# SumitTarafder/Figbird

Hardware: AMD Instinct MI355X
Metric: gaps/sec (+ filled-bases/sec), synthetic 1e5-gap set recipe, jump-library fill pass (higher is better)
Workload: dtype f64

## Files before the change

figbird_amd/csrc/fig_abi.hip:

```cpp
#include <hip/hip_runtime.h>

#include <algorithm>
#include <cstdio>
#include <cstdlib>
#include <cstring>
#include <new>
#include <vector>
#include <chrono>
#include <thread>
#include <mutex>

#include "../../include/figbird_hip.h"
#include "fig_engine.h"
#include "fig_pack.h"
#include "fig_abi_host.h"
#include "fig_quality.h"
#include "fig_quality_host.h"

#ifdef FIG_PROF
#define FIG_PROF_BEGIN() const unsigned long long _k0 = __builtin_readcyclecounter()
#define FIG_PROF_FLUSH() do { if (E.lane == 0) { atomicAdd(&B.counters[FIG_CNT_WAIT], E.wait_cycles); atomicAdd(&B.counters[FIG_CNT_WAVE], (unsigned long long)__builtin_readcyclecounter() - _k0); \
    for (int i = 0; i < FIG_PROF_SLOTS; i++) if (E.prof[i]) atomicAdd(&B.counters[i < FIG_PROF_SPLIT ? FIG_CNT_PROF_LO + i : FIG_CNT_PROF_HI + (i - FIG_PROF_SPLIT)], E.prof[i]); } } while (0)
#else
#define FIG_PROF_BEGIN() ((void)0)
#define FIG_PROF_FLUSH() ((void)0)
#endif

FIG_D void fig_eng_init(FigEng &E, const FigDevModel &M, const FigDevBatch &B, const FigKernArgs &A, bool lds_tab, FigScr &work) {
    fig_eng_ident(E, threadIdx.x, blockDim.x, 64);
    E.M = &M; E.B = &B;
    E.flops = 0; E.mle_alg = 0; E.mle_exec = 0; E.wait_cycles = 0;
    for (int i = 0; i < FIG_PROF_SLOTS; i++) E.prof[i] = 0;
    unsigned char *slab = B.scratch + (long long)blockIdx.x * B.scratch_stride;
    fig_scratch_layout(slab, B.capG, B.capR, B.capP, B.capC, B.capW, B.capE, &work);
    E.scr = work;
    fig_eng_carve(E, M, A, lds_tab);
}

FIG_D void fig_kernel_begin(FigEng &E, const FigDevModel &M, const FigDevBatch &B, const FigKernArgs &A, bool lds_tab, FigScr &work) {
    fig_eng_init(E, M, B, A, lds_tab, work);
    if (blockIdx.x == 0 && threadIdx.x == 0) B.queue_head[A.qsel ^ 1] = 0;
}

FIG_D int fig_queue_pop(FigEng &E, const FigDevBatch &B, const FigKernArgs &A) {
    if (E.tid == 0) E.S->bc_i = atomicAdd(B.queue_head + A.qsel, 1);
    __syncthreads();
    const int qi = E.S->bc_i;
    __syncthreads();
    return qi;
}

template <typename T> struct FigItemSrc { const T *v; int first, end; };
FIG_D FigItemSrc<int32_t> fig_src_order(const FigDevBatch &B, const FigKernArgs &A) { return {B.order, A.q_begin, A.q_end}; }

template <typename Src, typename Body>
FIG_D void fig_pop_loop(FigEng &E, const FigDevBatch &B, const FigKernArgs &A, Src src, Body body) {
    while (true) {
        const int qi = fig_queue_pop(E, B, A);
        const auto s = src();
        if (s.first + qi >= s.end) break;
        body(s.v[s.first + qi]);
    }
}

FIG_D void fig_kernel_flush(const FigEng &E, const FigDevBatch &B) {
    if (E.flops) atomicAdd(&B.counters[FIG_CNT_FLOPS], E.flops);
    if (E.mle_alg) atomicAdd(&B.counters[FIG_CNT_MLE_ALG], E.mle_alg);
    if (E.lane == 0 && E.mle_exec) atomicAdd(&B.counters[FIG_CNT_MLE_EXEC], E.mle_exec);
}

template <bool LDS_TAB, int NT>
__global__ void __launch_bounds__(NT, (NT <= 256 ? 2 : 1)) fig_fill_kernel(FigDevModel M, FigDevBatch B, FigKernArgs A) {
    FigEng E; FigScr work;
    fig_kernel_begin(E, M, B, A, LDS_TAB, work);
    FIG_PROF_BEGIN();
    fig_pop_loop(E, B, A, [&] { return fig_src_order(B, A); }, [&](int gi) { fig_item_fill<LDS_TAB>(E, work, gi); });
    FIG_PROF_FLUSH();
    fig_kernel_flush(E, B);
}

template <bool LDS_TAB, int NT>
__global__ void __launch_bounds__(NT, (NT <= 256 ? 2 : 1)) fig_begin_kernel(FigDevModel M, FigDevBatch B, FigKernArgs A) {
    FigEng E; FigScr work;
    fig_kernel_begin(E, M, B, A, LDS_TAB, work);
    fig_pop_loop(E, B, A, [&] { return fig_src_order(B, A); }, [&](int gi) { fig_item_begin<LDS_TAB>(E, work, gi); });
    fig_kernel_flush(E, B);
}

template <bool LDS_TAB, int NT>
__global__ void __launch_bounds__(NT, (NT <= 256 ? 2 : 1)) fig_probe_kernel(FigDevModel M, FigDevBatch B, FigKernArgs A) {
    FigEng E; FigScr work;
    fig_kernel_begin(E, M, B, A, LDS_TAB, work);
    fig_pop_loop(E, B, A, [&] { return fig_src_order(B, A); }, [&](int gi) { fig_item_probe<LDS_TAB>(E, work, gi); });
}

static_assert(sizeof(FigItem) == sizeof(int4) && sizeof(FigEntry) == sizeof(int4), "item records travel as int4");
template <bool LDS_TAB, int NT>
__global__ void __launch_bounds__(NT, (NT <= 256 ? 2 : 1)) fig_eval_kernel(FigDevModel M, FigDevBatch B, FigKernArgs A, const int4 *items, int n_items) {
    FigEng E; FigScr work;
    fig_kernel_begin(E, M, B, A, LDS_TAB, work);
    FIG_PROF_BEGIN();
    fig_pop_loop(E, B, A, [&] { return FigItemSrc<FigItem>{(const FigItem *)items, 0, n_items}; }, [&](FigItem it) { fig_item_eval<LDS_TAB>(E, work, it); });
    FIG_PROF_FLUSH();
    fig_kernel_flush(E, B);
}

__global__ void __launch_bounds__(64) fig_replay_kernel(FigDevModel M, FigDevBatch B, const int4 *entries, int n) {
    if ((int)blockIdx.x >= n) return;
    FigEng E{}; FigScr work{};
    fig_eng_ident(E, threadIdx.x, blockDim.x, 64);
    E.M = &M; E.B = &B; E.nteams = 1; E.S = (FigState *)fig_lds;
    const FigEntry en = ((const FigEntry *)entries)[blockIdx.x];
    fig_item_replay(E, work, en);
}

template <bool LDS_TAB, int NT>
__global__ void __launch_bounds__(NT, (NT <= 256 ? 2 : 1)) fig_end_kernel(FigDevModel M, FigDevBatch B, FigKernArgs A, const int *list, int n) {
    FigEng E; FigScr work;
    fig_kernel_begin(E, M, B, A, LDS_TAB, work);
    fig_pop_loop(E, B, A, [&] { return FigItemSrc<int>{list, 0, n}; }, [&](int gi) { fig_item_end<LDS_TAB>(E, work, gi); });
    fig_kernel_flush(E, B);
}

__global__ void __launch_bounds__(256) fig_stream_kernel(FigDevModel M, FigDevBatch B, uint32_t *out) {
    for (long long gi = blockIdx.x; gi < B.n_gaps; gi += gridDim.x) {
        const FigDevGap &g = B.gaps[gi];
        const int L = M.L;
        const long long n = (long long)((g.nU + FIG_SH_C - 1) / FIG_SH_C) * L * (FIG_SH_C / 2);
        for (long long i = threadIdx.x; i < n; i += blockDim.x) {
            const int sp = (int)(i % (FIG_SH_C / 2));
            const long long cj = i / (FIG_SH_C / 2);
            const int j = (int)(cj % L);
            uint32_t v = 0;
            for (int h = 0; h < 2; h++) {
                const long long r = (cj / L) * FIG_SH_C + 2 * sp + h;
                unsigned e = 0x1000u | FIG_SH_ONE;
                if (r < g.nU) {
                    const long long idx = g.uBase + r;
                    const int len = B.u.len[idx], aux = B.u.aux[idx];
                    if (len == L && !(aux & 2)) {
                        const uint32_t w = B.packed[B.u.woff[idx] + (j >> 4)];
                        e = 0x1000u | (2u * (4u * (unsigned)(aux & 1) + ((w >> ((j & 15) * 2)) & 3u)));
                    }
                }
                v |= e << (16 * h);
            }
            out[g.streamOff + i] = v;
        }
    }
}

#define FIG_HIP(call) do { hipError_t _e = (call); if (_e != hipSuccess) { ctx->last_hip = (int)_e; return FIG_EHIP; } } while (0)

struct DevBuf { void *p = nullptr; };

struct FigTmpBufs {
    std::vector<void *> bufs;
    ~FigTmpBufs() { for (void *p : bufs) hipFree(p); }
    void *alloc(size_t n) { void *p = nullptr; if (hipMalloc(&p, n ? n : 8) != hipSuccess) return nullptr; bufs.push_back(p); return p; }
};

struct FigLane { hipStream_t stream = nullptr; hipEvent_t done = nullptr; int32_t *queue_head = nullptr; uint8_t *scratch = nullptr; FigItem *d_items = nullptr; FigEntry *d_entries = nullptr; size_t cap = 0;
                 FigGapCtl *h_ctl = nullptr; FigItem *h_items = nullptr; FigEntry *h_entries = nullptr; int qsel = 0; };

struct fig_ctx {
    int device = 0;
    hipStream_t stream = nullptr;
    hipEvent_t ev0 = nullptr, ev1 = nullptr;
    int n_cu = 0;
    int last_hip = 0;
    bool have_model = false;
    FigDevModel dm;
    DevBuf d_model_tabs;
    fig_model hm;
    bool have_batch = false;
    FigDevBatch db;
    std::vector<int32_t> h_order;
    struct Cls { FigLaunchClass c; int blocks; int capacity; };
    std::vector<Cls> classes;
    std::vector<DevBuf> bufs;
    int64_t n_gaps = 0, n_ureads = 0, n_preads = 0, str_total = 0;
    std::vector<int64_t> h_str_off;
    int nslots = 32;
    std::vector<FigLane> lanes;
    fig_stats stats;
    int sh_on = FIG_SH_SC;
    std::vector<uint8_t> h_ot;
    uint8_t *d_ot = nullptr;
};

static int dev_alloc(fig_ctx *ctx, size_t bytes, void **out) {
    DevBuf b;
    if (bytes == 0) bytes = 8;
    hipError_t e = hipMalloc(&b.p, bytes);
    if (e != hipSuccess) { ctx->last_hip = (int)e; return FIG_ENOMEM; }
    ctx->bufs.push_back(b);
    *out = b.p;
    return FIG_OK;
}

template <typename T>
static int dev_upload(fig_ctx *ctx, const std::vector<T> &v, const T **out) {
    void *p = nullptr;
    int rc = dev_alloc(ctx, v.size() * sizeof(T), &p);
    if (rc) return rc;
    if (!v.empty()) {
        hipError_t e = hipMemcpyAsync(p, v.data(), v.size() * sizeof(T), hipMemcpyHostToDevice, ctx->stream);
        if (e != hipSuccess) { ctx->last_hip = (int)e; return FIG_EHIP; }
    }
    *out = (const T *)p;
    return FIG_OK;
}

extern "C" int fig_version(void) { return FIG_ABI_VERSION; }

extern "C" const char *fig_strerror(int code) { return fig_strerror_text(code); }

extern "C" int fig_ctx_create(int device_ordinal, fig_ctx **out) {
    if (!out) return FIG_EINVAL;
    *out = nullptr;
    static std::once_flag env_once;
    std::call_once(env_once, [] { setenv("GPU_MAX_HW_QUEUES", "8", 0); });
    int n = 0;
    if (hipGetDeviceCount(&n) != hipSuccess || n <= 0) return FIG_ENODEV;
    if (device_ordinal < 0 || device_ordinal >= n) return FIG_ENODEV;
    if (hipSetDevice(device_ordinal) != hipSuccess) return FIG_ENODEV;
    hipDeviceProp_t prop;
    if (hipGetDeviceProperties(&prop, device_ordinal) != hipSuccess) return FIG_ENODEV;
    fig_ctx *ctx = new (std::nothrow) fig_ctx();
    if (!ctx) return FIG_ENOMEM;
    ctx->device = device_ordinal;
    ctx->n_cu = prop.multiProcessorCount > 0 ? prop.multiProcessorCount : 256;
    if (hipStreamCreate(&ctx->stream) != hipSuccess || hipEventCreate(&ctx->ev0) != hipSuccess || hipEventCreate(&ctx->ev1) != hipSuccess) {
        delete ctx;
        return FIG_EHIP;
    }
    memset(&ctx->stats, 0, sizeof(ctx->stats));
    ctx->sh_on = fig_knobs_from_env(0).sh_on;
    *out = ctx;
    return FIG_OK;
}

static void free_batch(fig_ctx *ctx) {
    for (auto &b : ctx->bufs) if (b.p) hipFree(b.p);
    ctx->bufs.clear();
    ctx->d_ot = nullptr;
    ctx->have_batch = false;
    ctx->classes.clear();
    for (auto &l : ctx->lanes) { if (l.stream) hipStreamDestroy(l.stream); if (l.done) hipEventDestroy(l.done); if (l.h_ctl) hipHostFree(l.h_ctl); if (l.h_items) hipHostFree(l.h_items); if (l.h_entries) hipHostFree(l.h_entries); }
    ctx->lanes.clear();
}

extern "C" void fig_batch_free(fig_ctx *ctx) {
    if (!ctx) return;
    hipSetDevice(ctx->device);
    free_batch(ctx);
}

extern "C" void fig_ctx_destroy(fig_ctx *ctx) {
    if (!ctx) return;
    hipSetDevice(ctx->device);
    free_batch(ctx);
    if (ctx->d_model_tabs.p) hipFree(ctx->d_model_tabs.p);
    if (ctx->ev0) hipEventDestroy(ctx->ev0);
    if (ctx->ev1) hipEventDestroy(ctx->ev1);
    if (ctx->stream) hipStreamDestroy(ctx->stream);
    delete ctx;
}

extern "C" int fig_ctx_set_model(fig_ctx *ctx, const fig_model *m) {
    if (!ctx) return FIG_EINVAL;
    if (int rc = fig_model_check(m)) return rc;
    hipSetDevice(ctx->device);
    free_batch(ctx);
    ctx->hm = *m;
    std::vector<double> all;
    FigModelOffsets o;
    fig_model_tables(m, all, o, ctx->dm);
    if (ctx->d_model_tabs.p) { hipFree(ctx->d_model_tabs.p); ctx->d_model_tabs.p = nullptr; }
    if (hipMalloc(&ctx->d_model_tabs.p, all.size() * sizeof(double)) != hipSuccess) return FIG_ENOMEM;
    if (hipMemcpy(ctx->d_model_tabs.p, all.data(), all.size() * sizeof(double), hipMemcpyHostToDevice) != hipSuccess) return FIG_EHIP;
    fig_model_point(ctx->dm, o, (const double *)ctx->d_model_tabs.p);
    ctx->have_model = true;
    return FIG_OK;
}

extern "C" int64_t fig_results_capacity(const fig_model *m, const fig_gap_batch *b) {
    if (!m || !b) return FIG_EINVAL;
    return fig_pack_results_capacity(m, b);
}

enum FigKind { FIG_K_FILL, FIG_K_BEGIN, FIG_K_EVAL, FIG_K_END, FIG_K_PROBE };

template <typename... P, typename... Args>
static hipError_t launch_one(void (*k)(P...), size_t lds, int nt, int blocks, hipStream_t stream, Args... args) {
    hipError_t e = hipFuncSetAttribute((const void *)k, hipFuncAttributeMaxDynamicSharedMemorySize, (int)lds);
    if (e != hipSuccess) return e;
    hipLaunchKernelGGL(k, dim3(blocks), dim3(nt), lds, stream, args...);
    return hipGetLastError();
}

template <bool LDS_TAB, int NT>
static hipError_t launch_kind(fig_ctx *ctx, const fig_ctx::Cls &c, const FigDevBatch &db, hipStream_t stream, FigKind kind, int blocks, const void *list, int n, int qsel) {
    const FigKernArgs A = fig_kargs_of(c.c, qsel, ctx->sh_on);
    switch (kind) {
        case FIG_K_FILL: return launch_one(fig_fill_kernel<LDS_TAB, NT>, c.c.lds, NT, blocks, stream, ctx->dm, db, A);
        case FIG_K_BEGIN: return launch_one(fig_begin_kernel<LDS_TAB, NT>, c.c.lds, NT, blocks, stream, ctx->dm, db, A);
        case FIG_K_PROBE: return launch_one(fig_probe_kernel<LDS_TAB, NT>, c.c.lds, NT, blocks, stream, ctx->dm, db, A);
        case FIG_K_EVAL: return launch_one(fig_eval_kernel<LDS_TAB, NT>, c.c.lds, NT, blocks, stream, ctx->dm, db, A, (const int4 *)list, n);
        case FIG_K_END: return launch_one(fig_end_kernel<LDS_TAB, NT>, c.c.lds, NT, blocks, stream, ctx->dm, db, A, (const int *)list, n);
    }
    return hipErrorInvalidValue;
}

static hipError_t launch_any(fig_ctx *ctx, const fig_ctx::Cls &c, const FigDevBatch &db, hipStream_t stream, FigKind kind, int blocks, const void *list, int n, int qsel = 0) {
    if (c.c.tiles > 0) return launch_kind<true, 512>(ctx, c, db, stream, kind, blocks, list, n, qsel);
    if (c.c.lds_tab) return c.c.nt == 256 ? launch_kind<true, 256>(ctx, c, db, stream, kind, blocks, list, n, qsel) : launch_kind<true, 512>(ctx, c, db, stream, kind, blocks, list, n, qsel);
    return launch_kind<false, 512>(ctx, c, db, stream, kind, blocks, list, n, qsel);
}

extern "C" int fig_batch_upload(fig_ctx *ctx, const fig_gap_batch *b) {
    if (!ctx || !b) return FIG_EINVAL;
    if (!ctx->have_model) return FIG_EINVAL;
    hipSetDevice(ctx->device);
    free_batch(ctx);
    const fig_model *m = &ctx->hm;
    hipEventRecord(ctx->ev0, ctx->stream);
    FigPacked K;
    int prc = fig_pack(m, b, sizeof(FigState), K);
    if (prc) return prc;
    int64_t ng = K.n_gaps;
    ctx->h_order = K.order; ctx->h_str_off = K.str_off;
    ctx->str_total = K.str_total; ctx->n_gaps = ng;
    ctx->n_ureads = (int64_t)K.u_pos.size(); ctx->n_preads = (int64_t)K.p_pos.size();
    ctx->classes.clear();
    const bool log = fig_knobs_from_env(0).log;
    for (const FigLaunchClass &lc : K.classes) {
        fig_ctx::Cls c;
        c.c = lc;
        int per_cu = (int)std::max<size_t>(1, std::min<size_t>((160 * 1024) / std::max<size_t>(lc.lds, 1), (size_t)(2048 / lc.nt)));
        per_cu = std::min(per_cu, 8);
        c.capacity = ctx->n_cu * per_cu;
        c.blocks = std::min<int>(lc.q_end - lc.q_begin, c.capacity);
        if (log) fprintf(stderr, "[figsched] class: capG=%d capGl=%d ncolE=%d Wcap=%d nt=%d nteams=%d lds_tab=%d tiles=%d tile_cols=%d lds=%zu gaps=%d per_cu=%d blocks=%d (FigState %zu B)\n",
                                             lc.capG, lc.capGl, lc.ncolE, lc.Wcap, lc.nt, lc.nteams, (int)lc.lds_tab, lc.tiles, lc.tile_cols, lc.lds, lc.q_end - lc.q_begin, per_cu, c.blocks, sizeof(FigState));
        ctx->classes.push_back(c);
    }
    int64_t stride = fig_scratch_layout(nullptr, K.capG, K.capR, K.capP, K.capC, K.capW, K.capE, nullptr);
    stride = (stride + 255) & ~255LL;

    FigDevBatch &db = ctx->db;
    memset(&db, 0, sizeof(db));
    db.n_gaps = ng;
    int rc;
#define UP(vec, field) do { rc = dev_upload(ctx, K.vec, &db.field); if (rc) return rc; } while (0)
    UP(gaps, gaps); UP(order, order); UP(packed, packed); UP(qual, qual); UP(flank, flank);
    UP(u_pos, u.pos); UP(u_aux, u.aux); UP(u_len, u.len); UP(u_woff, u.woff);
    UP(p_pos, p.pos); UP(p_aux, p.aux); UP(p_clip, p.clip); UP(p_ref, p.refpos); UP(p_len, p.len); UP(p_woff, p.woff); UP(p_qoff, p.qoff);
#undef UP
    db.u.clip = nullptr; db.u.refpos = nullptr; db.u.qoff = nullptr;
    void *p;
    if (m->unmapped_flag) {
        if ((rc = dev_alloc(ctx, (size_t)K.stream_total * 4, &p))) return rc;
        db.ustream = (const uint32_t *)p;
        FIG_HIP(hipMemsetD32Async((hipDeviceptr_t)p, (int)(((0x1000u | FIG_SH_ONE) << 16) | (0x1000u | FIG_SH_ONE)), (size_t)K.stream_total, ctx->stream));
        if (ng > 0) {
            hipLaunchKernelGGL(fig_stream_kernel, dim3((unsigned)std::min<int64_t>(ng, 4096)), dim3(256), 0, ctx->stream, ctx->dm, db, (uint32_t *)p);
            FIG_HIP(hipGetLastError());
        }
    }
    if ((rc = dev_alloc(ctx, (size_t)ng * 4, &p))) return rc; db.filled_len = (int32_t *)p;
    if ((rc = dev_alloc(ctx, (size_t)ng * 4, &p))) return rc; db.gaptofill = (int32_t *)p;
    if ((rc = dev_alloc(ctx, (size_t)K.str_total, &p))) return rc; db.str = (char *)p;
    if ((rc = dev_alloc(ctx, 64 * (ctx->classes.size() + 1), &p))) return rc; db.queue_head = (int32_t *)p;
    if ((rc = dev_alloc(ctx, FIG_CNT_N * sizeof(unsigned long long), &p))) return rc; db.counters = (unsigned long long *)p;
    size_t total_blocks = 0;
    for (const fig_ctx::Cls &c : ctx->classes) total_blocks += (size_t)c.capacity;
    if ((rc = dev_alloc(ctx, (size_t)stride * std::max<size_t>(total_blocks, 1), &p))) return rc; db.scratch = (uint8_t *)p;
    if ((rc = dev_alloc(ctx, (size_t)K.persist_total + 256, &p))) return rc; db.persist = (uint8_t *)p;
    if ((rc = dev_alloc(ctx, (size_t)std::max<int64_t>(ng, 1) * sizeof(FigGapCtl), &p))) return rc; db.gapctl = (FigGapCtl *)p;
    if ((rc = dev_alloc(ctx, (size_t)std::max<int64_t>(ng, 1), &p))) return rc; ctx->d_ot = (uint8_t *)p; db.ot_preset = ctx->d_ot;
    ctx->h_ot = K.ot_preset;
    FIG_HIP(hipMemcpyAsync(ctx->d_ot, ctx->h_ot.data(), (size_t)std::max<int64_t>(ng, 1), hipMemcpyHostToDevice, ctx->stream));
    ctx->nslots = K.nslots;
    {   size_t blk = 0;
        for (size_t ci = 0; ci < ctx->classes.size(); ci++) {
            const fig_ctx::Cls &c = ctx->classes[ci];
            ctx->lanes.push_back(FigLane());
            FigLane &l = ctx->lanes.back();
            if (hipStreamCreate(&l.stream) != hipSuccess || hipEventCreateWithFlags(&l.done, hipEventDisableTiming) != hipSuccess) return FIG_EHIP;
            l.queue_head = db.queue_head + 16 * (ci + 1);
            l.scratch = db.scratch + (size_t)stride * blk; blk += (size_t)c.capacity;
            l.cap = (size_t)std::max(c.c.q_end - c.c.q_begin, 1) * (size_t)(K.nslots + 1);
            if ((rc = dev_alloc(ctx, l.cap * sizeof(FigItem), &p))) return rc; l.d_items = (FigItem *)p;
            if ((rc = dev_alloc(ctx, l.cap * sizeof(FigEntry), &p))) return rc; l.d_entries = (FigEntry *)p;
            if (hipHostMalloc((void **)&l.h_ctl, (size_t)std::max<int64_t>(ng, 1) * sizeof(FigGapCtl), hipHostMallocDefault) != hipSuccess) return FIG_ENOMEM;
            if (hipHostMalloc((void **)&l.h_items, l.cap * sizeof(FigItem), hipHostMallocDefault) != hipSuccess) return FIG_ENOMEM;
            if (hipHostMalloc((void **)&l.h_entries, l.cap * sizeof(FigEntry), hipHostMallocDefault) != hipSuccess) return FIG_ENOMEM;
        }
    }
    db.scratch_stride = stride;
    db.capG = K.capG; db.capR = K.capR; db.capP = K.capP; db.capC = K.capC; db.capW = K.capW; db.capE = K.capE;
    db.n_ureads = ctx->n_ureads;
    FIG_HIP(hipMemsetAsync(db.counters, 0, FIG_CNT_N * sizeof(unsigned long long), ctx->stream));
    FIG_HIP(hipMemsetAsync(db.queue_head, 0, 64 * (ctx->classes.size() + 1), ctx->stream));
    hipEventRecord(ctx->ev1, ctx->stream);
    FIG_HIP(hipStreamSynchronize(ctx->stream));
    float ms = 0; hipEventElapsedTime(&ms, ctx->ev0, ctx->ev1);
    ctx->stats.h2d_ms = ms;
    ctx->stats.packed_bytes = K.packed_bytes();
    ctx->have_batch = true;
    if (!K.ot_given && m->partial_flag && ng > 0 && (rc = fig_ot_carry_measured(ctx, ng))) { free_batch(ctx); return rc; }
    return FIG_OK;
}

extern "C" int fig_batch_probe_reach(fig_ctx *ctx, uint8_t *reach) {
    if (!ctx || !reach || !ctx->have_batch) return FIG_EINVAL;
    hipSetDevice(ctx->device);
    const int64_t ng = ctx->n_gaps;
    memset(reach, 0, (size_t)ng);
    if (!ctx->hm.partial_flag || ng == 0) return FIG_OK;
    FigDevBatch db = ctx->db;
    fig_batch_clear_planes(db);
    FIG_HIP(hipMemsetAsync(db.gapctl, 0, (size_t)ng * sizeof(FigGapCtl), ctx->stream));
    for (const fig_ctx::Cls &c : ctx->classes) {
        FIG_HIP(hipMemsetAsync(db.queue_head, 0, 8, ctx->stream));
        FIG_HIP(launch_any(ctx, c, db, ctx->stream, FIG_K_PROBE, c.blocks, nullptr, 0));
    }
    std::vector<FigGapCtl> ctl((size_t)ng);
    FIG_HIP(hipMemcpyAsync(ctl.data(), db.gapctl, (size_t)ng * sizeof(FigGapCtl), hipMemcpyDeviceToHost, ctx->stream));
    FIG_HIP(hipStreamSynchronize(ctx->stream));
    for (int64_t g = 0; g < ng; g++) reach[g] = ctl[g].reach ? 1 : 0;
    return FIG_OK;
}

extern "C" int fig_batch_set_ot_preset(fig_ctx *ctx, const uint8_t *preset) {
    if (!ctx || !preset || !ctx->have_batch) return FIG_EINVAL;
    hipSetDevice(ctx->device);
    const int64_t ng = ctx->n_gaps;
    for (int64_t g = 0; g < ng; g++) ctx->h_ot[(size_t)g] = preset[g] ? 1 : 0;
    if (ng > 0) { FIG_HIP(hipMemcpy(ctx->d_ot, ctx->h_ot.data(), (size_t)ng, hipMemcpyHostToDevice)); }
    return FIG_OK;
}

static int run_class_parallel(fig_ctx *ctx, const fig_ctx::Cls &c, FigLane &ln, const FigKnobs &knobs) {
    FigDevBatch db = ctx->db;
    db.queue_head = ln.queue_head; db.scratch = ln.scratch;
    hipStream_t stream = ln.stream;
    hipSetDevice(ctx->device);
    int nl = 0;
    hipError_t e;
    auto fail = [&](hipError_t er) { ctx->last_hip = (int)er; return -1; };
    const int capacity = std::max(1, c.capacity);
    auto launch = [&](FigKind kind, int n_work, const void *list) {
        hipError_t er = launch_any(ctx, c, db, stream, kind, std::min(capacity, n_work), list, n_work, ln.qsel);
        ln.qsel ^= 1; nl++;
        return er;
    };
    if ((e = launch(FIG_K_BEGIN, c.c.q_end - c.c.q_begin, nullptr)) != hipSuccess) return fail(e);
    FigGapCtl *ctl = ln.h_ctl;
    const size_t ctl_bytes = (size_t)ctx->n_gaps * sizeof(FigGapCtl);
    const std::vector<int> ids(ctx->h_order.begin() + c.c.q_begin, ctx->h_order.begin() + c.c.q_end);
    FigRound R;
    auto now = [] { return std::chrono::duration<double, std::milli>(std::chrono::steady_clock::now().time_since_epoch()).count(); };
    const double t_start = now();
    double t_prev = now(); int round = 0, last_items = 0, last_active = 0, last_chunk = 0, n_active_max = 0;
    while (true) {
        if ((e = hipMemcpyAsync(ctl, db.gapctl, ctl_bytes, hipMemcpyDeviceToHost, stream)) != hipSuccess) return fail(e);
        if ((e = hipStreamSynchronize(stream)) != hipSuccess) return fail(e);
        fig_plan_round(ids, ctl, capacity, c.c.nsplit, ctx->nslots, knobs.minc, knobs.ipw, n_active_max, R);
        if (knobs.log) { double t = now(); fprintf(stderr, "[figsched] capG=%d round %d: active=%d chunk=%d items=%d blocks=%d  %.1f ms\n", c.c.capG, round, last_active, last_chunk, last_items, capacity, t - t_prev); t_prev = t; }
        round++;
        if (R.n_active == 0) break;
        if (ln.cap < R.items.size() || ln.cap < R.entries.size()) return fail(hipErrorOutOfMemory);
        const int n_items = (int)R.items.size(), n_ent = (int)R.entries.size();
        const size_t items_bytes = R.items.size() * sizeof(FigItem), ent_bytes = R.entries.size() * sizeof(FigEntry);
        last_items = n_items; last_active = R.n_active; last_chunk = R.chunk;
        if (n_items > 0) {
            memcpy(ln.h_items, R.items.data(), items_bytes);
            if ((e = hipMemcpyAsync(ln.d_items, ln.h_items, items_bytes, hipMemcpyHostToDevice, stream)) != hipSuccess) return fail(e);
            if ((e = launch(FIG_K_EVAL, n_items, ln.d_items)) != hipSuccess) return fail(e);
        }
        memcpy(ln.h_entries, R.entries.data(), ent_bytes);
        if ((e = hipMemcpyAsync(ln.d_entries, ln.h_entries, ent_bytes, hipMemcpyHostToDevice, stream)) != hipSuccess) return fail(e);
        hipLaunchKernelGGL(fig_replay_kernel, dim3(n_ent), dim3(64), sizeof(FigState) + 64, stream, ctx->dm, db, (const int4 *)ln.d_entries, n_ent);
        if ((e = hipGetLastError()) != hipSuccess) return fail(e);
        nl++;
    }
    std::vector<int> endlist;
    for (int g : ids) if (ctl[g].status == FIG_GAP_LOOP_DONE) endlist.push_back(g);
    if (!endlist.empty()) {
        if ((e = hipStreamSynchronize(stream)) != hipSuccess) return fail(e);
        memcpy(ln.h_items, endlist.data(), endlist.size() * sizeof(int));
        if ((e = hipMemcpyAsync(ln.d_items, ln.h_items, endlist.size() * sizeof(int), hipMemcpyHostToDevice, stream)) != hipSuccess) return fail(e);
        if ((e = launch(FIG_K_END, (int)endlist.size(), ln.d_items)) != hipSuccess) return fail(e);
        if (knobs.log) { const double t0 = now(); hipStreamSynchronize(stream); fprintf(stderr, "[figsched] capG=%d end kernel: %d gaps, %.1f ms (lane done at %.1f ms since its first round)\n", c.c.capG, (int)endlist.size(), now() - t0, now() - t_start); }
    }
    return nl;
}

extern "C" int fig_fill_resident(fig_ctx *ctx, fig_gap_results *out) { return fig_fill_resident_ex(ctx, out, nullptr); }

extern "C" int fig_fill_resident_ex(fig_ctx *ctx, fig_gap_results *out, const fig_gap_support *sup) {
    if (!ctx || !out || !ctx->have_batch) return FIG_EINVAL;
    if (!out->filled_len || !out->gaptofill || !out->str_off || (!out->str && ctx->str_total > 0)) return FIG_EINVAL;
    if (sup && (!sup->counts || !sup->origin)) return FIG_EINVAL;
    hipSetDevice(ctx->device);
    int64_t ng = ctx->n_gaps;
    FigDevBatch &db = ctx->db;
    FigTmpBufs tmp;
    std::vector<int32_t> hsup(sup ? (size_t)ctx->str_total * 5 : 0);
    const std::vector<FigPlane> planes = fig_fill_planes(db, ctx->n_ureads + ctx->n_preads, ctx->str_total, out, sup, hsup.data());
    auto clear = [&](void *p, int v, size_t n) { return n ? hipMemsetAsync(p, v, n, ctx->stream) : hipSuccess; };
    auto fetch = [&](void *dst, const void *src, size_t n) { return n ? hipMemcpyAsync(dst, src, n, hipMemcpyDeviceToHost, ctx->stream) : hipSuccess; };
    for (const FigPlane &pl : planes) {
        if (!(*pl.dev = tmp.alloc(pl.bytes))) return FIG_ENOMEM;
        if (pl.fill >= 0) FIG_HIP(clear(*pl.dev, pl.fill, pl.bytes));
    }
    FIG_HIP(clear(db.counters, 0, FIG_CNT_N * sizeof(unsigned long long)));
    FIG_HIP(clear(db.queue_head, 0, 64 * (ctx->classes.size() + 1)));
    for (auto &l : ctx->lanes) l.qsel = 0;
    FIG_HIP(clear(db.filled_len, 0, (size_t)std::max<int64_t>(ng, 1) * 4));
    FIG_HIP(clear(db.gaptofill, 0, (size_t)std::max<int64_t>(ng, 1) * 4));
    FIG_HIP(clear(db.str, 'N', (size_t)ctx->str_total));
    FIG_HIP(clear(db.gapctl, 0, (size_t)std::max<int64_t>(ng, 1) * sizeof(FigGapCtl)));
    FIG_HIP(hipEventRecord(ctx->ev0, ctx->stream));
    int nl = 0;
    const FigKnobs knobs = fig_knobs_from_env(ctx->dm.unmapped);
    if (knobs.seq) {
        for (const fig_ctx::Cls &c : ctx->classes) {
            FIG_HIP(clear(db.queue_head, 0, 4));
            FIG_HIP(launch_any(ctx, c, db, ctx->stream, FIG_K_FILL, c.blocks, nullptr, 0));
            nl++;
        }
    } else {
        const size_t nc = ctx->classes.size();
        std::vector<int> rcs(nc, 0);
        for (size_t ci = 0; ci < nc; ci++) FIG_HIP(hipStreamWaitEvent(ctx->lanes[ci].stream, ctx->ev0, 0));
        if (nc <= 1 || knobs.lanes_serial) {
            for (size_t ci = 0; ci < nc; ci++) rcs[ci] = run_class_parallel(ctx, ctx->classes[ci], ctx->lanes[ci], knobs);
        } else {
            std::vector<std::thread> th;
            for (size_t ci = 0; ci < nc; ci++) th.emplace_back([&, ci] { rcs[ci] = run_class_parallel(ctx, ctx->classes[ci], ctx->lanes[ci], knobs); });
            for (auto &t : th) t.join();
        }
        for (size_t ci = 0; ci < nc; ci++) {
            if (rcs[ci] < 0) { hipDeviceSynchronize(); return FIG_EHIP; }
            nl += rcs[ci];
            FIG_HIP(hipEventRecord(ctx->lanes[ci].done, ctx->lanes[ci].stream));
            FIG_HIP(hipStreamWaitEvent(ctx->stream, ctx->lanes[ci].done, 0));
        }
    }
    FIG_HIP(hipEventRecord(ctx->ev1, ctx->stream)); FIG_HIP(hipStreamSynchronize(ctx->stream));
    float ms = 0; FIG_HIP(hipEventElapsedTime(&ms, ctx->ev0, ctx->ev1));
    ctx->stats.kernel_ms = ms; ctx->stats.n_launches = nl;
    FIG_HIP(hipEventRecord(ctx->ev0, ctx->stream));
    std::vector<char> hstr((size_t)ctx->str_total);
    unsigned long long cnt[FIG_CNT_N] = {0};
    FIG_HIP(fetch(out->filled_len, db.filled_len, (size_t)ng * 4)); FIG_HIP(fetch(out->gaptofill, db.gaptofill, (size_t)ng * 4));
    FIG_HIP(fetch(hstr.data(), db.str, (size_t)ctx->str_total));
    FIG_HIP(fetch(cnt, db.counters, sizeof(cnt)));
    for (const FigPlane &pl : planes) FIG_HIP(fetch(pl.host, *pl.dev, pl.bytes));
    FIG_HIP(hipEventRecord(ctx->ev1, ctx->stream)); FIG_HIP(hipStreamSynchronize(ctx->stream));
    FIG_HIP(hipEventElapsedTime(&ms, ctx->ev0, ctx->ev1));
    ctx->stats.d2h_ms = ms;
#ifdef FIG_PROF
    { auto prof = [&](int i) { return cnt[i < FIG_PROF_SPLIT ? FIG_CNT_PROF_LO + i : FIG_CNT_PROF_HI + (i - FIG_PROF_SPLIT)]; };
      const unsigned long long wave = cnt[FIG_CNT_WAVE];
      const char *nm[14] = {"A.wait", "B.wait", "-", "M.finish", "PR.pre", "PR.estep", "PR.mid", "PR.mle", "PR.post", "A.chain", "A.logexp", "A.work", "B.work", "M.chains"};
      for (int i = 0; i < 14; i++) fprintf(stderr, "[figprof] %-9s %8.1f Gcycles = %5.1f %% of wave-cycles\n", nm[i], prof(i) / 1e9, wave ? 100.0 * prof(i) / wave : 0.0);
      const char *mn[4] = {"M.setup", "M.hint", "M.rounds", "M.surv"};
      for (int i = 0; i < 4; i++) fprintf(stderr, "[figprof] %-9s %8.1f Gcycles = %5.1f %% of wave-cycles\n", mn[i], prof(14 + i) / 1e9, wave ? 100.0 * prof(14 + i) / wave : 0.0);
      fprintf(stderr, "[figprof] raw slots:"); for (int i = 0; i < FIG_PROF_SLOTS; i++) fprintf(stderr, " %d:%.1f", i, prof(i) / 1e9); fprintf(stderr, "\n");
      fprintf(stderr, "[figprof] barrier wait %.3f of %.3f wave-Gcycles = %.1f %%\n", cnt[FIG_CNT_WAIT] / 1e9, wave / 1e9, wave ? 100.0 * cnt[FIG_CNT_WAIT] / wave : 0.0); }
#endif
    if (knobs.log) fprintf(stderr, "[figsched] useful flops %.4g, speculative evaluations executed %.4g (%.1f %% discarded)\n", (double)cnt[FIG_CNT_FLOPS], (double)cnt[FIG_CNT_SPEC], cnt[FIG_CNT_SPEC] ? 100.0 * (1.0 - ((double)cnt[FIG_CNT_FLOPS] / (double)cnt[FIG_CNT_SPEC])) : 0.0);
    fig_stats_from_counters(cnt, ctx->stats);
    int rc = fig_compact_results(ng, hstr.data(), ctx->h_str_off.data(), out);
    if (!rc && sup) fig_compact_support(ng, hsup.data(), ctx->h_str_off.data(), out, sup->counts);
    return rc;
}

extern "C" int fig_batch_quality(fig_ctx *ctx, const fig_gap_results *f, const int32_t *origin, fig_gap_quality *q) {
    if (!ctx || !f || !q || !ctx->have_batch || !ctx->have_model) return FIG_EINVAL;
    if (!f->filled_len || !f->str_off || !f->draw_pos || !f->draw_isz || !f->draw_len || !q->loglik || !q->phred || !q->state) return FIG_EINVAL;
    hipSetDevice(ctx->device);
    const int64_t ng = ctx->n_gaps, nr = ctx->n_ureads + ctx->n_preads;
    if (f->str_off[0] < 0) return FIG_EINVAL;
    for (int64_t g = 0; g < ng; g++) if (f->str_off[g + 1] < f->str_off[g]) return FIG_EINVAL;
    const int64_t total = f->str_off[ng];
    if (total > 0 && !f->str) return FIG_EINVAL;
    const FigDevBatch &db = ctx->db;
    const int L = ctx->dm.L;
    std::vector<FigDevGap> hg((size_t)ng);
    std::vector<double> he((size_t)L), home((size_t)L), tabs((size_t)fig_quality_tab_doubles(L));
    if (ng > 0) FIG_HIP(hipMemcpyAsync(hg.data(), db.gaps, (size_t)ng * sizeof(FigDevGap), hipMemcpyDeviceToHost, ctx->stream));
    FIG_HIP(hipMemcpyAsync(he.data(), ctx->dm.e, (size_t)L * sizeof(double), hipMemcpyDeviceToHost, ctx->stream));
    FIG_HIP(hipMemcpyAsync(home.data(), ctx->dm.ome1, (size_t)L * sizeof(double), hipMemcpyDeviceToHost, ctx->stream));
    FIG_HIP(hipStreamSynchronize(ctx->stream));
    fig_quality_tables(L, he.data(), home.data(), ctx->dm.T, tabs.data(), tabs.data() + L, tabs.data() + 2 * L);
    std::vector<int32_t> list, ncol((size_t)std::max<int64_t>(ng, 1), 0);
    std::vector<uint8_t> part((size_t)std::max<int64_t>(ng, 1), 0);
    int64_t cols = 0, reads = 0;
    for (int64_t g = 0; g < ng; g++) {
        const int32_t n = f->filled_len[g], lu = f->draw_len[2 * g], lp = f->draw_len[2 * g + 1];
        q->state[g] = fig_quality_gap_on(n, lu, lp, origin != nullptr, origin ? origin[g] : 0);
        if (q->state[g] != FIG_QUAL_ON) continue;
        if (n > (1 << 30) || f->str_off[g] + n > f->str_off[g + 1]) return FIG_EINVAL;
        const bool p = lp >= 0;
        const int64_t base = p ? ctx->n_ureads + hg[(size_t)g].pBase : hg[(size_t)g].uBase, cnt = p ? hg[(size_t)g].nP : hg[(size_t)g].nU;
        if (base < 0 || cnt < 0 || base + cnt > nr) return FIG_EINVAL;
        const int64_t drawn = fig_quality_check_placements(f->draw_pos + base, cnt);
        if (drawn < 0) return FIG_EINVAL;
        list.push_back((int32_t)g); ncol[(size_t)g] = n; part[(size_t)g] = p ? 1 : 0;
        cols += n; reads += drawn;
    }
    float ms = 0;
    if (total > 0) memset(q->loglik, 0, (size_t)total * 4 * sizeof(double));
    if (total > 0) memset(q->phred, 0, (size_t)total);
    if (!list.empty()) {
        FigTmpBufs tmp;
        auto up = [&](const void *src, size_t bytes) -> void * {
            void *p = tmp.alloc(bytes);
            if (p && bytes && hipMemcpyAsync(p, src, bytes, hipMemcpyHostToDevice, ctx->stream) != hipSuccess) return nullptr;
            return p;
        };
        FigQualArgs A;
        A.gaps = db.gaps; A.u_len = db.u.len; A.u_aux = db.u.aux; A.p_len = db.p.len; A.u_woff = db.u.woff; A.p_woff = db.p.woff;
        A.packed = db.packed; A.n_ureads = ctx->n_ureads; A.L = L;
        A.draw_pos = (const int32_t *)up(f->draw_pos, (size_t)nr * 4);
        A.list = (const int32_t *)up(list.data(), list.size() * 4);
        A.ncol = (const int32_t *)up(ncol.data(), (size_t)ng * 4);
        A.partial = (const uint8_t *)up(part.data(), (size_t)ng);
        A.str_off = (const int64_t *)up(f->str_off, (size_t)(ng + 1) * 8);
        A.tabs = (const double *)up(tabs.data(), tabs.size() * sizeof(double));
        A.loglik = (double *)tmp.alloc((size_t)total * 4 * sizeof(double));
        if (!A.draw_pos || !A.list || !A.ncol || !A.partial || !A.str_off || !A.tabs || !A.loglik) { hipStreamSynchronize(ctx->stream); return FIG_ENOMEM; }
        FIG_HIP(hipMemsetAsync(A.loglik, 0, (size_t)total * 4 * sizeof(double), ctx->stream));
        FIG_HIP(hipEventRecord(ctx->ev0, ctx->stream));
        hipLaunchKernelGGL(fig_quality_kernel, dim3((unsigned)list.size()), dim3(FIG_Q_NT), 0, ctx->stream, A);
        FIG_HIP(hipGetLastError());
        FIG_HIP(hipEventRecord(ctx->ev1, ctx->stream));
        FIG_HIP(hipMemcpyAsync(q->loglik, A.loglik, (size_t)total * 4 * sizeof(double), hipMemcpyDeviceToHost, ctx->stream));
        FIG_HIP(hipStreamSynchronize(ctx->stream));
        FIG_HIP(hipEventElapsedTime(&ms, ctx->ev0, ctx->ev1));
    }
    for (int32_t g : list)
        for (int64_t i = f->str_off[g], e = f->str_off[g] + ncol[(size_t)g]; i < e; i++) q->phred[i] = fig_quality_phred(q->loglik + i * 4, f->str[i]);
    if (fig_knobs_from_env(ctx->dm.unmapped).log)
        fprintf(stderr, "[figqual] gaps on %zu of %lld, columns %lld, reads %lld, kernel %.3f ms\n", list.size(), (long long)ng, (long long)cols, (long long)reads, ms);
    return FIG_OK;
}

extern "C" int fig_fill_gaps(fig_ctx *ctx, const fig_gap_batch *batch, fig_gap_results *out) { return fig_fill_gaps_once(ctx, batch, out); }

extern "C" int fig_get_stats(const fig_ctx *ctx, fig_stats *out) {
    if (!ctx || !out) return FIG_EINVAL;
    *out = ctx->stats;
    return FIG_OK;
}
```

figbird_amd/csrc/fig_abi_host.h:

```cpp
#ifndef FIG_ABI_HOST_H
#define FIG_ABI_HOST_H
#include <algorithm>
#include <cmath>
#include <cstdlib>
#include <cstring>
#include <vector>
#include "../../include/figbird_hip.h"
#include "fig_types.h"
#include "fig_gaprules.h"

static_assert(FIG_ORG_NONE == FIG_SUP_NONE && FIG_ORG_FINAL == FIG_SUP_FINAL && FIG_ORG_ORIGINAL == FIG_SUP_ORIGINAL && FIG_ORG_TIEBREAK == FIG_SUP_TIEBREAK,
              "the engine's path mask (fig_types.h) is fig_gap_support::origin");

static inline const char *fig_strerror_text(int code) {
    switch (code) {
        case FIG_OK: return "ok";
        case FIG_EINVAL: return "invalid argument";
        case FIG_ENODEV: return "no usable HIP device (libfighip has no CPU path)";
        case FIG_ENOMEM: return "out of memory";
        case FIG_EHIP: return "HIP runtime error";
        case FIG_ENOSPC: return "result string buffer too small";
        case FIG_EUNSUP: return "input outside the supported envelope";
        default: return "unknown error";
    }
}

static inline int fig_model_check(const fig_model *m) {
    if (!m || !m->error_pos_dist || !m->in_pos_dist || !m->del_pos_dist || !m->insert_len_dist_smoothed) return FIG_EINVAL;
    if (m->max_read_length <= 0 || m->max_read_length > FIG_MAX_READLEN) return FIG_EUNSUP;
    if (m->max_insert_size <= 0) return FIG_EINVAL;
    if (m->partial_flag && m->unmapped_flag) return FIG_EUNSUP;
    if (m->insert_threshold_min < 0 || m->insert_threshold_max >= m->max_insert_size + 1) return FIG_EINVAL;
    return FIG_OK;
}

struct FigModelOffsets { size_t e, pairs, m3, insd, qtab, ome; };

static void fig_model_tables(const fig_model *m, std::vector<double> &all, FigModelOffsets &o, FigDevModel &dm) {
    const int L = m->max_read_length;
    std::vector<double> h_e(m->error_pos_dist, m->error_pos_dist + L), h_ome(L), h_m3(L);
    for (int k = 0; k < L; k++) {
        volatile double a = 1 - m->error_pos_dist[k];
        h_ome[k] = a;
        volatile double b = 1 - m->error_pos_dist[k] - m->in_pos_dist[k] - m->del_pos_dist[k];
        h_m3[k] = b;
    }
    std::vector<double> h_insd(m->insert_len_dist_smoothed, m->insert_len_dist_smoothed + m->max_insert_size);
    h_insd.push_back(0.0);
    std::vector<double> h_qtab(256);
    for (int c = 0; c < 256; c++) { int Q = c - 33; h_qtab[c] = pow(10, -Q / 10.0); }
    std::vector<double> pairs((size_t)8 * L);
    for (int k = 0; k < L; k++) {
        pairs[2 * k] = h_ome[k]; pairs[2 * k + 1] = h_e[k];
        pairs[2 * L + 2 * k] = h_ome[L - 1 - k]; pairs[2 * L + 2 * k + 1] = h_e[L - 1 - k];
        pairs[4 * L + 2 * k] = h_m3[k]; pairs[4 * L + 2 * k + 1] = h_e[k];
        pairs[6 * L + 2 * k] = h_m3[L - 1 - k]; pairs[6 * L + 2 * k + 1] = h_e[L - 1 - k];
    }
    all.clear();
    o.e = 0; all.insert(all.end(), h_e.begin(), h_e.end()); while (all.size() % 8) all.push_back(0);
    o.pairs = all.size(); all.insert(all.end(), pairs.begin(), pairs.end()); while (all.size() % 8) all.push_back(0);
    o.m3 = all.size(); all.insert(all.end(), h_m3.begin(), h_m3.end()); while (all.size() % 8) all.push_back(0);
    o.insd = all.size(); all.insert(all.end(), h_insd.begin(), h_insd.end()); while (all.size() % 8) all.push_back(0);
    o.qtab = all.size(); all.insert(all.end(), h_qtab.begin(), h_qtab.end());
    o.ome = all.size(); all.insert(all.end(), h_ome.begin(), h_ome.end());
    dm.L = L; dm.Tmin = m->insert_threshold_min; dm.Tmax = m->insert_threshold_max; dm.cutoff = m->gap_prob_cutoff;
    dm.partial_flag = m->partial_flag; dm.unmapped = m->unmapped_flag; dm.script_itr = m->script_itr; dm.D = m->max_distance;
    dm.read_length = m->read_length; dm.neg_overlap = m->neg_overlap; dm.partial_len = m->partial_len; dm.unm_limit = m->unm_limit;
    dm.max_insert = m->max_insert_size;
    for (int i = 0; i < 25; i++) dm.T[i] = m->error_type_probs[i];
    dm.fmm_up = fig_model_fmm(m);
}

static inline void fig_model_point(FigDevModel &dm, const FigModelOffsets &o, const double *d) {
    dm.e = d + o.e; dm.ome = d + o.pairs; dm.m3 = d + o.m3; dm.insd = d + o.insd; dm.qtab = d + o.qtab;
    dm.ome1 = d + o.ome;
}

static inline void fig_batch_clear_planes(FigDevBatch &db) {
    db.dbg_n_cand = nullptr; db.dbg_cand_i = nullptr; db.dbg_cand_lik = nullptr; db.dbg_max_cand = 0; db.dbg_n_place = nullptr;
    db.draw_pos = db.draw_isz = db.draw_len = nullptr;
    db.dbg_counts = db.dbg_read_maxlv = nullptr; db.dbg_plane_cols = db.dbg_plane_reads = 0;
    db.sup_counts = db.sup_origin = nullptr;
}

struct FigPlane { void **dev; void *host; size_t bytes; int fill; };

static std::vector<FigPlane> fig_fill_planes(FigDevBatch &db, int64_t n_reads, int64_t str_total, const fig_gap_results *out, const fig_gap_support *sup, int32_t *sup_host) {
    std::vector<FigPlane> pl;
    auto add = [&](auto *&dev, void *host, size_t bytes, int fill) { pl.push_back(FigPlane{(void **)&dev, host, bytes, fill}); };
    const size_t ng = (size_t)db.n_gaps, nr = (size_t)n_reads;
    fig_batch_clear_planes(db);
    if (out->dbg_n_cand && out->dbg_cand_i && out->dbg_cand_lik && out->dbg_max_cand > 0) {
        const size_t nc = ng * out->dbg_max_cand;
        db.dbg_max_cand = out->dbg_max_cand;
        add(db.dbg_n_cand, out->dbg_n_cand, ng * 4, 0);
        add(db.dbg_cand_i, out->dbg_cand_i, nc * 12, -1);
        add(db.dbg_cand_lik, out->dbg_cand_lik, nc * 8, -1);
        if (out->dbg_n_place) add(db.dbg_n_place, out->dbg_n_place, ng * 4, 0);
        if (out->dbg_counts && out->dbg_plane_cols > 0) { db.dbg_plane_cols = out->dbg_plane_cols; add(db.dbg_counts, out->dbg_counts, nc * out->dbg_plane_cols * 5 * 8, 0); }
        if (out->dbg_read_maxlv && out->dbg_plane_reads > 0) { db.dbg_plane_reads = out->dbg_plane_reads; add(db.dbg_read_maxlv, out->dbg_read_maxlv, nc * out->dbg_plane_reads * 8, 0); }
    }
    if (out->draw_pos && out->draw_isz && out->draw_len) {
        add(db.draw_pos, out->draw_pos, nr * 4, -1);
        add(db.draw_isz, out->draw_isz, nr * 4, 0);
        add(db.draw_len, out->draw_len, ng * 8, -1);
    }
    if (sup) {
        add(db.sup_counts, sup_host, (size_t)str_total * 5 * 4, 0);
        add(db.sup_origin, sup->origin, ng * 4, 0);
    }
    return pl;
}

static inline void fig_stats_from_counters(const unsigned long long *cnt, fig_stats &st) {
    st.place_calls = (int64_t)cnt[FIG_CNT_PLACE];
    st.alg_flops = (double)cnt[FIG_CNT_FLOPS]; st.spec_flops = (double)cnt[FIG_CNT_SPEC];
    st.mle_alg_flops = (double)cnt[FIG_CNT_MLE_ALG]; st.mle_exec_flops = (double)cnt[FIG_CNT_MLE_EXEC];
}

static FigKernArgs fig_kargs_of(const FigLaunchClass &c, int qsel, int sh_on) {
    FigKernArgs A;
    A.capG = c.capG; A.capGl = c.capGl; A.ncolE = c.ncolE; A.Wcap = c.Wcap; A.nteams = c.nteams;
    A.q_begin = c.q_begin; A.q_end = c.q_end; A.qsel = qsel;
    A.tiles = c.tiles; A.tile_step = c.tile_step; A.tile_cols = c.tile_cols; A.tiled_max = c.tiled_max;
    A.sh_on = sh_on;
    return A;
}

static int fig_ot_carry_measured(fig_ctx *ctx, int64_t ng) {
    std::vector<uint8_t> reach((size_t)ng, 0), preset((size_t)ng, 0);
    int rc;
    if ((rc = fig_batch_probe_reach(ctx, reach.data()))) return rc;
    std::vector<int64_t> ids((size_t)ng);
    for (int64_t g = 0; g < ng; g++) ids[(size_t)g] = g;
    fig_ot_carry(ids, reach.data(), preset.data());
    return fig_batch_set_ot_preset(ctx, preset.data());
}

static int fig_compact_results(int64_t ng, const char *src, const int64_t *src_off, fig_gap_results *out) {
    int64_t need = 0;
    for (int64_t g = 0; g < ng; g++) need += out->filled_len[g] > 0 ? out->filled_len[g] : 0;
    if (need > out->str_capacity) return FIG_ENOSPC;
    int64_t o = 0;
    for (int64_t g = 0; g < ng; g++) {
        out->str_off[g] = o;
        int n = out->filled_len[g];
        if (n > 0) { memcpy(out->str + o, src + src_off[g], (size_t)n); o += n; }
    }
    out->str_off[ng] = o;
    return FIG_OK;
}

static void fig_compact_support(int64_t ng, const int32_t *src, const int64_t *src_off, const fig_gap_results *out, int32_t *dst) {
    for (int64_t g = 0; g < ng; g++) {
        int n = out->filled_len[g];
        if (n > 0) memcpy(dst + out->str_off[g] * 5, src + src_off[g] * 5, (size_t)n * 5 * sizeof(int32_t));
    }
}

static int fig_fill_gaps_once(fig_ctx *ctx, const fig_gap_batch *batch, fig_gap_results *out) {
    int rc = fig_batch_upload(ctx, batch);
    if (rc) return rc;
    rc = fig_fill_resident(ctx, out);
    fig_batch_free(ctx);
    return rc;
}

struct FigKnobs {
    bool seq;
    bool lanes_serial;
    bool log;
    int minc;
    double ipw;
    int sh_on;
};

static FigKnobs fig_knobs_from_env(int unmapped) {
    FigKnobs k;
    const char *sched = getenv("FIG_SCHED"), *ser = getenv("FIG_LANES"), *mc = getenv("FIG_MIN_CHUNK"), *ipw = getenv("FIG_ITEMS_PER_WG");
    const char *ev = getenv("FIG_ESTEP"), *sc = getenv("FIG_SH_CHUNKS");
    k.seq = sched && strcmp(sched, "seq") == 0;
    k.lanes_serial = ser && strcmp(ser, "serial") == 0;
    k.log = getenv("FIG_SCHED_LOG") != nullptr;
    k.minc = mc ? std::max(1, atoi(mc)) : 16;
    k.ipw = ipw ? std::max(1.0, atof(ipw)) : (unmapped ? 12.0 : 6.0);
    k.sh_on = (ev && !strcmp(ev, "pair")) ? 0 : (sc ? std::max(1, std::min(FIG_SH_SC, atoi(sc))) : FIG_SH_SC);
    return k;
}

struct FigRound { std::vector<FigItem> items; std::vector<FigEntry> entries; int chunk = 0, n_active = 0; };

static void fig_plan_round(const std::vector<int> &ids, const FigGapCtl *ctl, int capacity, int nsplit, int slots_cap, int minc, double ipw_base,
                           int &n_active_max, FigRound &R) {
    R.items.clear(); R.entries.clear();
    R.chunk = 0; R.n_active = 0;
    for (int g : ids) if (ctl[g].status == FIG_GAP_MORE) R.n_active++;
    if (R.n_active == 0) return;
    long long rem_total = 0;
    for (int g : ids) if (ctl[g].status == FIG_GAP_MORE) rem_total += std::max(0, ctl[g].range - ctl[g].j);
    n_active_max = std::max(n_active_max, R.n_active);
    const double ipw = ipw_base * std::min(8.0, std::max(1.0, n_active_max / 96.0));
    const double share = rem_total > 0 ? (ipw * capacity / (double)std::max(1, nsplit)) / (double)rem_total : 1.0;
    const double target = ipw * capacity / (double)std::max(1, nsplit);
    long long total = 0;
    for (int g : ids) {
        if (ctl[g].status != FIG_GAP_MORE) continue;
        if ((double)total >= 1.25 * target) break;
        int j = ctl[g].j, range = ctl[g].range;
        int want = (int)std::ceil((range - j) * share);
        want = std::min(std::max(want, minc), slots_cap);
        int n = std::max(0, std::min(want, range - j));
        R.chunk = std::max(R.chunk, n);
        total += n;
        R.entries.push_back(FigEntry{g, n, 0, 0});
    }
    for (const FigEntry &en : R.entries)
        for (int k = en.n - 1; k >= 0; k--) R.items.push_back(FigItem{en.gap, ctl[en.gap].j + k, k, 0});
}

#endif
```

figbird_amd/csrc/fig_engine.h:

```cpp
#ifndef FIG_ENGINE_H
#define FIG_ENGINE_H

#include "fig_types.h"

#ifdef FIG_EMU
#include <cmath>
#include <cstring>
#define FIG_D static inline
#define FIG_NOINLINE
#define FIG_HD static inline
#define FIG_SYNC() ((void)0)
FIG_D double fig_log10(double x) { return log10(x); }
FIG_D double fig_log(double x) { return log(x); }
FIG_D double fig_exp(double x) { return exp(x); }
FIG_D double fig_pow10(double x) { return pow(10, x); }
FIG_D int fig_atomic_add_i32(int *p, int v) { int o = *p; *p += v; return o; }
FIG_D void fig_atomic_max_i32(int *p, int v) { if (v > *p) *p = v; }
FIG_D int fig_atomic_fetch_add_i32(int *p, int v) { int o = *p; *p += v; return o; }
FIG_D void fig_atomic_min_i32(int *p, int v) { if (v < *p) *p = v; }
FIG_D void fig_atomic_or_i32(int *p, int v) { *p |= v; }
FIG_D void fig_atomic_add_u64(unsigned long long *p, unsigned long long v) { *p += v; }
FIG_D unsigned long long fig_shfl_down_u64(unsigned long long v, int off) { (void)v; (void)off; return 0; }
#else
#include <hip/hip_runtime.h>
#define FIG_D __device__ static
#define FIG_NOINLINE __attribute__((noinline))
#define FIG_HD __host__ __device__ static
#ifdef FIG_PROF
#define FIG_SYNC() do { unsigned long long _bt = __builtin_readcyclecounter(); __syncthreads(); E.wait_cycles += __builtin_readcyclecounter() - _bt; } while (0)
#else
#define FIG_SYNC() __syncthreads()
#endif
FIG_D double fig_log10(double x) { return log10(x); }
FIG_D double fig_log(double x) { return log(x); }
FIG_D double fig_exp(double x) { return exp(x); }
FIG_D double fig_pow10(double x) { return pow(10.0, x); }
FIG_D int fig_atomic_add_i32(int *p, int v) { return atomicAdd(p, v); }
FIG_D void fig_atomic_max_i32(int *p, int v) { atomicMax(p, v); }
FIG_D int fig_atomic_fetch_add_i32(int *p, int v) { return atomicAdd(p, v); }
FIG_D void fig_atomic_min_i32(int *p, int v) { atomicMin(p, v); }
FIG_D void fig_atomic_or_i32(int *p, int v) { atomicOr(p, v); }
FIG_D void fig_atomic_add_u64(unsigned long long *p, unsigned long long v) { atomicAdd(p, v); }
FIG_D unsigned long long fig_shfl_down_u64(unsigned long long v, int off) { return __shfl_down(v, off, 64); }
#endif

#define FIG_NOPOS 0x7fffffff
#define FIG_PLB_TEAMS 8
#define FIG_PLB_BYTES (FIG_PLB_TEAMS * 64 * 4)

#if defined(FIG_PROF) && !defined(FIG_EMU)
#define FIG_T0(E) unsigned long long _fig_t = __builtin_readcyclecounter()
#define FIG_TICK(E, slot) do { unsigned long long _n = __builtin_readcyclecounter(); (E).prof[slot] += _n - _fig_t; _fig_t = _n; } while (0)
#define FIG_COUNT(E, slot, n) do { (E).prof[slot] += (n); } while (0)
#else
#define FIG_COUNT(E, slot, n) do { } while (0)
#define FIG_T0(E) do { } while (0)
#define FIG_TICK(E, slot) do { } while (0)
#endif

#ifdef FIG_EMU
static double *fig_lds = nullptr;
#define FIG_RFL(x) (x)
typedef const uint32_t *fig_cu32p;
typedef const double *fig_cdp;
typedef double *fig_gdp;
typedef const double *fig_gcdp;
typedef const uint32_t *fig_gcu32p;
typedef const unsigned char *fig_gcu8p;
typedef const unsigned char *fig_lcu8p;
#else
extern __shared__ __attribute__((aligned(16))) double fig_lds[];
#define FIG_RFL(x) __builtin_amdgcn_readfirstlane(x)
typedef const uint32_t __attribute__((address_space(4))) *fig_cu32p;
typedef const double __attribute__((address_space(4))) *fig_cdp;
typedef double __attribute__((address_space(1))) *fig_gdp;
typedef const double __attribute__((address_space(1))) *fig_gcdp;
typedef const uint32_t __attribute__((address_space(1))) *fig_gcu32p;
typedef const unsigned char __attribute__((address_space(1))) *fig_gcu8p;
typedef const unsigned char __attribute__((address_space(3))) *fig_lcu8p;
#endif

struct alignas(16) FigPQ { double p, q; };

struct FigLoop {
    int inr, range, gapMin, j, gapEstimate, maxGapEstimate, finalize_flag;
    int fill_or_not, same_count, same_thresh, stuckCount, side_flag, less_read_flag;
    int prev_best, curr_best, prev_u, curr_u, sec_same, sec_same2;
    int done, need_orig;
    int ev_iters, ev_side_break, ev_fill;
    double maxLikelihood, secondMaxLikelihood, prevlikelihood, likelihood;
};

struct FigState {
    int G, ncols;
    int left, right;
    int side_limit; long long end_pos_max;
    int valid_count, invalid_count, partial_read_count;
    double region_perct, region_perct_max;
    int partial_read_len, rep_flag, one_side_repeat_flag, large_gap_flag, comp_count;
    int left_max, right_min, discont_or_not;
    int psr_temp[2], psr_final[2];
    int umaxleftf, umaxrightf, ucoverf;
    int num_itr, overlap_threshold, gaptofill;
    int gl_len, gr_len, pl_len, pr_len;
    int cons_len, best_len, cur_len, prev_len, orig_len;
    unsigned char gap_left[32], gap_right[32];
    unsigned char partial_left[100], partial_right[100];
    double FP[6][5], FQ[6][5];
    double red_v[16]; int red_i[16];
    double bc_d; int bc_i, bc_j;
    int ibuf[8];
    double lik;
    int ctl[8];
    int tm_lo[16], tm_hi[16], tm_len[16], tm_tis0[16], tm_dir[16];
    int tm_aux[16]; long long tm_woff[16];
    double wv_v[32]; int wv_o[32];
    short sh_lo[FIG_SH_SC * FIG_SH_C], sh_hi[FIG_SH_SC * FIG_SH_C];
    int sh_tis0[FIG_SH_SC * FIG_SH_C];
    unsigned sh_woff[FIG_SH_SC * FIG_SH_C];
    unsigned char sh_len[FIG_SH_SC * FIG_SH_C], sh_aux[FIG_SH_SC * FIG_SH_C];
    unsigned sh_irr[16], sh_pad;
    int mle_next, pad_mn;
    int fin_i[8];
    FigLoop L;
    unsigned long long flops_useful; int n_place, sup_any;
    int dbg_j, sup_origin;
};

struct FigTrip { int v[3]; };



struct FigScr {
    double *cnt;
    double *ncnt;
    double *tmp;
    int *pc;
    int *nci;
    unsigned char *accf;
    unsigned char *mdone;
    int *cov;
    int *region;
    unsigned char *cons, *best, *cur, *prev, *orig;
    unsigned char *colchar;
    unsigned char *mark, *saved;
    double *maxlv;
    int *frp;
    int *org;
    int *fin;
    FigTrip *sortbuf;
    int *hint;
    int *hint_e;
    double *hval;
    int *repeatflag;
    int *ppos_org;
    int *pflag;
    int *prf;
    int *lcross, *rcross; unsigned char *smflag;
    int *used_read_arr; int *lrmd;
    FigPQ *pqg; double *q4g;
    double *wg;
};

FIG_HD long long fig_align8(long long x) { return (x + 15) & ~15LL; }

FIG_HD long long fig_scratch_layout(unsigned char *base, int capG, int capR, int capP, int capC, int capW, int capE, FigScr *s) {
    long long o = 0;
#define FIG_CARVE(field, type, count) do { if (s) s->field = (type *)(base + o); o = fig_align8(o + (long long)sizeof(type) * (count)); } while (0)
    FIG_CARVE(cnt, double, 5LL * capG);
    FIG_CARVE(ncnt, double, 5LL * capG);
    FIG_CARVE(tmp, double, 5LL * capG);
    FIG_CARVE(pqg, FigPQ, 4LL * capE);
    FIG_CARVE(q4g, double, capE);
    FIG_CARVE(wg, double, capW);
    FIG_CARVE(maxlv, double, capR > capP ? capR : capP);
    FIG_CARVE(hval, double, capR);
    FIG_CARVE(pc, int, 4LL * capG);
    FIG_CARVE(nci, int, 5LL * capG);
    FIG_CARVE(cov, int, capG);
    FIG_CARVE(region, int, 2LL * capG + 16);
    FIG_CARVE(frp, int, 2LL * capR);
    FIG_CARVE(org, int, 2LL * capR);
    FIG_CARVE(fin, int, 2LL * capR);
    FIG_CARVE(sortbuf, FigTrip, capR);
    FIG_CARVE(hint, int, capR);
    FIG_CARVE(hint_e, int, capR);
    FIG_CARVE(repeatflag, int, 3LL * capP);
    FIG_CARVE(ppos_org, int, 3LL * capP);
    FIG_CARVE(pflag, int, 2LL * capP);
    FIG_CARVE(prf, int, 3LL * capP);
    FIG_CARVE(lcross, int, capP);
    FIG_CARVE(rcross, int, capP);
    FIG_CARVE(used_read_arr, int, capC);
    FIG_CARVE(lrmd, int, 2LL * capC);
    FIG_CARVE(cons, unsigned char, capG + 8);
    FIG_CARVE(best, unsigned char, capG + 8);
    FIG_CARVE(cur, unsigned char, capG + 8);
    FIG_CARVE(prev, unsigned char, capG + 8);
    FIG_CARVE(orig, unsigned char, capG + 8);
    FIG_CARVE(colchar, unsigned char, capG + 8);
    FIG_CARVE(mark, unsigned char, capR + 8);
    FIG_CARVE(saved, unsigned char, capR + 8);
    FIG_CARVE(accf, unsigned char, capR + 8);
    FIG_CARVE(mdone, unsigned char, capR + 8);
    FIG_CARVE(smflag, unsigned char, capP + 8);
#undef FIG_CARVE
    return o;
}

struct FigEng {
    int tid, nt;
    const FigDevModel *M;
    const FigDevBatch *B;
    const FigDevGap *g;
    FigState *S;
    FigScr scr;
    FigPQ *pq; double *q4;
    int ncolE, xoff;
    int off_pq, off_q4, off_w;
    int off_plb;
    int pq_lds, w_lds;
    int lds_tw;
    int tiles, tile_step, tile_cols;
    double *wbuf;
    int Wcap, nteams;
    int sh_on;
    int lane, wave, nw, wsz;
    const double *kt_fwd, *kt_rev;
    const double *mt_fwd, *mt_rev;
    unsigned char *rb;
    uint32_t *plb;
    unsigned char *gs;
    int capG;
    unsigned long long flops;
    unsigned long long mle_alg;
    unsigned long long mle_exec;
    unsigned long long wait_cycles;
    unsigned long long prof[FIG_PROF_SLOTS];
};

FIG_D void fig_eng_ident(FigEng &E, unsigned tid, unsigned nt, unsigned wsz) {
    E.tid = (int)tid; E.nt = (int)nt;
    E.lane = (int)(tid % wsz); E.wave = (int)(tid / wsz); E.nw = (int)((nt + wsz - 1) / wsz); E.wsz = (int)wsz;
}

struct FigKernArgs { int capG, capGl, ncolE, Wcap, nteams, q_begin, q_end, qsel, tiles, tile_step, tile_cols, tiled_max, sh_on; };

FIG_D long long fig_eng_carve(FigEng &E, const FigDevModel &M, const FigKernArgs &A, bool lds_tab) {
    E.capG = A.capG;
    E.ncolE = A.ncolE; E.xoff = M.L - 1; E.Wcap = A.Wcap; E.nteams = A.nteams; E.sh_on = A.sh_on;
    long long off = 0;
    E.pq_lds = lds_tab; E.w_lds = lds_tab;
    E.tiles = A.tiles; E.tile_step = A.tile_step; E.tile_cols = A.tile_cols;
    if (lds_tab && A.tiles > 0) {
        E.pq_lds = 0;
        E.off_pq = 0; E.off_q4 = 8 * A.tile_cols; E.off_w = 9 * A.tile_cols;
        off = 9LL * A.tile_cols + (long long)A.nteams * A.Wcap;
        { const long long mle = FIG_TILED_MLE_DOUBLES(A.ncolE, (int)E.nw); if (mle > off && mle <= A.tiled_max) off = mle; }
        E.pq = E.scr.pqg; E.q4 = E.scr.q4g; E.wbuf = E.scr.wg;
    } else if (lds_tab) {
        E.off_pq = 0; E.off_q4 = 8 * A.ncolE; E.off_w = 9 * A.ncolE;
        off = 9LL * A.ncolE + (long long)A.nteams * A.Wcap;
        E.pq = (FigPQ *)(fig_lds + E.off_pq); E.q4 = fig_lds + E.off_q4; E.wbuf = fig_lds + E.off_w;
    } else {
        E.off_pq = E.off_q4 = E.off_w = 0;
        E.pq = E.scr.pqg; E.q4 = E.scr.q4g; E.wbuf = E.scr.wg;
    }
    E.S = (FigState *)(fig_lds + off); E.lds_tw = (int)off;
    unsigned char *bp = (unsigned char *)(E.S + 1);
    E.gs = bp; bp += ((A.capGl + 7) & ~7);
    E.rb = bp; bp += ((FIG_MAX_READLEN + 8 + 15) & ~15);
    E.plb = (uint32_t *)bp; E.off_plb = (int)((double *)bp - fig_lds);
    E.kt_fwd = M.ome; E.kt_rev = M.ome + 2 * M.L; E.mt_fwd = M.ome + 4 * M.L; E.mt_rev = M.ome + 6 * M.L;
    return off * 8 + (long long)sizeof(FigState) + ((A.capGl + 7) & ~7) + ((FIG_MAX_READLEN + 8 + 15) & ~15) + FIG_PLB_BYTES;
}

FIG_D int fig_read_code(const uint32_t *packed, long long woff, int len, int j) {
    int nw2 = (len + 15) >> 4;
    uint32_t w = packed[woff + (j >> 4)];
    uint32_t m = packed[woff + nw2 + (j >> 5)];
    int c = (w >> ((j & 15) * 2)) & 3;
    return ((m >> (j & 31)) & 1) ? 4 : c;
}

FIG_D int fig_flank_l(const FigEng &E, int k) {
    if (k > FIG_FLANK) return 4;
    return ((fig_gcu8p)E.B->flank)[E.g->flankOff + (k - 1)];
}
FIG_D int fig_flank_r(const FigEng &E, int k) {
    if (k >= FIG_FLANK) return 4;
    return ((fig_gcu8p)E.B->flank)[E.g->flankOff + FIG_FLANK + k];
}

FIG_D void fig_stage_read(FigEng &E, const FigDevReads &R, long long idx) {
    int len = R.len[idx];
    long long woff = R.woff[idx];
    for (int j = E.tid; j < len; j += E.nt) E.rb[j] = (unsigned char)fig_read_code(E.B->packed, woff, len, j);
}

FIG_D int fig_load_read(const FigEng &E, const FigDevReads &R, long long idx, unsigned char *dst) {
    int len = R.len[idx];
    long long woff = R.woff[idx];
    for (int j = 0; j < len; j++) dst[j] = (unsigned char)fig_read_code(E.B->packed, woff, len, j);
    return len;
}

struct FigBest { double v; int o; };

FIG_D int fig_ovl(int o, int len, int G) { int a = o > 0 ? o : 0, b = o + len < G ? o + len : G; return b > a ? b - a : 0; }

FIG_D FigBest fig_best_merge(FigBest a, FigBest b) {
    if (b.o == FIG_NOPOS) return a;
    if (a.o == FIG_NOPOS) return b;
    if (b.v > a.v || (b.v == a.v && b.o < a.o)) return b;
    return a;
}

FIG_D FigBest fig_block_best(FigEng &E, FigBest x) {
#ifdef FIG_EMU
    return x;
#else
    for (int off = 32; off > 0; off >>= 1) {
        FigBest y;
        y.v = __shfl_down(x.v, off, 64);
        y.o = __shfl_down(x.o, off, 64);
        x = fig_best_merge(x, y);
    }
    int wave = E.tid >> 6, nw = (E.nt + 63) >> 6;
    if (nw == 1) {
        x.v = __shfl(x.v, 0, 64);
        x.o = __shfl(x.o, 0, 64);
        return x;
    }
    FIG_SYNC();
    if ((E.tid & 63) == 0) { E.S->red_v[wave] = x.v; E.S->red_i[wave] = x.o; }
    FIG_SYNC();
    FigBest r; r.v = E.S->red_v[0]; r.o = E.S->red_i[0];
    for (int w = 1; w < nw; w++) { FigBest y; y.v = E.S->red_v[w]; y.o = E.S->red_i[w]; r = fig_best_merge(r, y); }
    return r;
#endif
}

FIG_D void fig_ise(FigEng &E) {
    FigState &S = *E.S;
    long long gs = E.g->gapStart, cl = E.g->contigLen;
    if (gs - S.left < 0) { S.left = (int)gs; if (S.side_limit > S.left) S.side_limit = S.left; }
    if (gs + S.G + S.right > cl) { S.right = (int)(cl - (gs + S.G)); if (S.side_limit > S.right) S.side_limit = S.right; }
    long long endPos = gs + S.G + S.right;
    if (endPos > S.end_pos_max) S.end_pos_max = endPos;
    S.ncols = S.G;
}

FIG_D void fig_flank_tables(FigEng &E) {
    FigState &S = *E.S;
    for (int c = 0; c < 6; c++) {
        double cnt[5] = {0, 0, 0, 0, 0};
        if (c < 5) cnt[c] = 1;
        double total = 0;
        for (int j = 0; j < 5; j++) total = total + cnt[j];
        double Ncount = cnt[4];
        double pr[5];
        for (int j = 0; j < 4; j++) pr[j] = (c < 5) ? ((cnt[j] + (Ncount / 4)) / total) : 0.0;
        pr[4] = 0;
        for (int j = 0; j < 5; j++) {
            double sum = 0;
            for (int k = 0; k < 4; k++) { if (j == k) continue; sum += pr[k] * E.M->T[k * 5 + j]; }
            S.FQ[c][j] = (c < 5) ? sum : 0.0;
            S.FP[c][j] = pr[j];
        }
    }
}

FIG_D int fig_col_kind(const FigEng &E, int x, int G, int left, int right) {
    if (x < 0) { if (x < -left) return -1; return fig_flank_l(E, -x); }
    if (x < G) return 6;
    if (x < G + right) return fig_flank_r(E, x - G);
    return 5;
}
FIG_D int fig_from_code(const FigEng &E, int x, int G, int left, int right) {
    if (x < 0) { if (x < -left) return 4; return fig_flank_l(E, -x); }
    if (x < G) return ((fig_lcu8p)E.gs)[x];
    if (x < G + right) return fig_flank_r(E, x - G);
    return 4;
}

FIG_D int fig_from_code_u(fig_gcu8p fl, fig_lcu8p gs, int x, int G, int left, int right) {
    if (x < 0) { if (x < -left) return 4; const int k = -x; return k > FIG_FLANK ? 4 : fl[k - 1]; }
    if (x < G) return gs[x];
    if (x < G + right) { const int k = x - G; return k >= FIG_FLANK ? 4 : fl[FIG_FLANK + k]; }
    return 4;
}

#define FIG_PQ(E, b, x) ((E).pq[(long long)(b) * (E).ncolE + (x) + (E).xoff])
#define FIG_Q4(E, x) ((E).q4[(x) + (E).xoff])
#ifdef FIG_EMU
FIG_D void fig_pq_set(const FigEng &E, int b, int x, FigPQ v) { FIG_PQ(E, b, x) = v; }
FIG_D FigPQ fig_pq_get(const FigEng &E, int b, int x) { return FIG_PQ(E, b, x); }
FIG_D void fig_pq_set_p(const FigEng &E, int b, int x, double v) { FIG_PQ(E, b, x).p = v; }
FIG_D void fig_pq_set_q(const FigEng &E, int b, int x, double v) { FIG_PQ(E, b, x).q = v; }
FIG_D double fig_pq_get_p(const FigEng &E, int b, int x) { return FIG_PQ(E, b, x).p; }
FIG_D void fig_q4_set(const FigEng &E, int x, double v) { FIG_Q4(E, x) = v; }
FIG_D double fig_q4_get(const FigEng &E, int x) { return FIG_Q4(E, x); }
#else
typedef double fig_d2v __attribute__((ext_vector_type(2)));
typedef fig_d2v __attribute__((address_space(3))) *fig_ld2p;
typedef fig_d2v __attribute__((address_space(1))) *fig_gd2p;
typedef double __attribute__((address_space(3))) *fig_ldp;
FIG_D void fig_pq_set(const FigEng &E, int b, int x, FigPQ v) {
    const long long i = (long long)b * E.ncolE + x + E.xoff;
    fig_d2v t; t.x = v.p; t.y = v.q;
    if (E.pq_lds) ((fig_ld2p)(fig_lds + E.off_pq))[i] = t; else ((fig_gd2p)E.pq)[i] = t;
}
FIG_D FigPQ fig_pq_get(const FigEng &E, int b, int x) {
    const long long i = (long long)b * E.ncolE + x + E.xoff;
    fig_d2v t;
    if (E.pq_lds) t = ((fig_ld2p)(fig_lds + E.off_pq))[i]; else t = ((fig_gd2p)E.pq)[i];
    FigPQ v; v.p = t.x; v.q = t.y;
    return v;
}
FIG_D void fig_pq_set_p(const FigEng &E, int b, int x, double v) {
    const long long i = (long long)b * E.ncolE + x + E.xoff;
    if (E.pq_lds) ((fig_ldp)(fig_lds + E.off_pq))[2 * i] = v; else ((fig_gdp)(double *)E.pq)[2 * i] = v;
}
FIG_D void fig_pq_set_q(const FigEng &E, int b, int x, double v) {
    const long long i = (long long)b * E.ncolE + x + E.xoff;
    if (E.pq_lds) ((fig_ldp)(fig_lds + E.off_pq))[2 * i + 1] = v; else ((fig_gdp)(double *)E.pq)[2 * i + 1] = v;
}
FIG_D double fig_pq_get_p(const FigEng &E, int b, int x) {
    const long long i = (long long)b * E.ncolE + x + E.xoff;
    if (E.pq_lds) return ((fig_ldp)(fig_lds + E.off_pq))[2 * i];
    return ((fig_gdp)(double *)E.pq)[2 * i];
}
FIG_D void fig_q4_set(const FigEng &E, int x, double v) {
    if (E.pq_lds) ((fig_ldp)(fig_lds + E.off_q4))[x + E.xoff] = v; else ((fig_gdp)E.q4)[x + E.xoff] = v;
}
FIG_D double fig_q4_get(const FigEng &E, int x) {
    if (E.pq_lds) return ((fig_ldp)(fig_lds + E.off_q4))[x + E.xoff];
    return ((fig_gdp)E.q4)[x + E.xoff];
}
#endif

FIG_D void fig_build_flank_pq(FigEng &E) {
    const FigState &S = *E.S;
    int G = S.G, left = S.left, right = S.right, L1 = E.xoff;
    int n = 2 * L1;
    for (int i = E.tid; i < n; i += E.nt) {
        int x = i < L1 ? i - L1 : G + (i - L1);
        if (x + E.xoff >= E.ncolE) continue;
        int c;
        if (x < 0) c = (-x <= left) ? fig_flank_l(E, -x) : 5;
        else c = (x - G < right) ? fig_flank_r(E, x - G) : 5;
        for (int b = 0; b < 4; b++) { FigPQ v; v.p = S.FP[c][b]; v.q = S.FQ[c][b]; fig_pq_set(E, b, x, v); }
        fig_q4_set(E, x, S.FQ[c][4]);
    }
}

FIG_D void fig_compute_probs(FigEng &E) {
    int n = E.S->ncols, cg = E.capG;
    const double *T = E.M->T;
    for (int x = E.tid; x < n; x += E.nt) {
        double c0 = E.scr.cnt[x], c1 = E.scr.cnt[cg + x], c2 = E.scr.cnt[2 * cg + x], c3 = E.scr.cnt[3 * cg + x], c4 = E.scr.cnt[4 * cg + x];
        double total = 0;
        total = total + c0; total = total + c1; total = total + c2; total = total + c3; total = total + c4;
        double pr[4];
        if (total) {
            double nq = c4 / 4;
            pr[0] = (c0 + nq) / total; pr[1] = (c1 + nq) / total; pr[2] = (c2 + nq) / total; pr[3] = (c3 + nq) / total;
        } else { pr[0] = pr[1] = pr[2] = pr[3] = .25; }
        for (int j = 0; j < 5; j++) {
            double sum = 0;
            for (int k = 0; k < 4; k++) { if (j == k) continue; sum += pr[k] * T[k * 5 + j]; }
            if (j < 4) { FigPQ v; v.p = pr[j]; v.q = sum; fig_pq_set(E, j, x, v); }
            else fig_q4_set(E, x, sum);
        }
    }
    fig_build_flank_pq(E);
}
FIG_D void fig_compute_errprobs_only(FigEng &E) {
    int n = E.S->ncols;
    const double *T = E.M->T;
    for (int x = E.tid; x < n; x += E.nt) {
        double pr[4];
        for (int j = 0; j < 4; j++) pr[j] = fig_pq_get_p(E, j, x);
        for (int j = 0; j < 5; j++) {
            double sum = 0;
            for (int k = 0; k < 4; k++) { if (j == k) continue; sum += pr[k] * T[k * 5 + j]; }
            if (j < 4) fig_pq_set_q(E, j, x, sum); else fig_q4_set(E, x, sum);
        }
    }
    fig_build_flank_pq(E);
}

FIG_D void fig_compute_sequence(FigEng &E, int check, int choice) {
    int n = E.S->ncols, cg = E.capG;
    const double *A = choice == 0 ? E.scr.cnt : E.scr.ncnt;
    for (int x = E.tid; x < n; x += E.nt) {
        double mx = 0; int mi = -1;
        for (int j = 0; j <= 4; j++) { double v = A[j * cg + x]; if (v > mx) { mx = v; mi = j; } }
        int coverage_flag = 1;
        if (check == 1) { int cv = (int)mx; E.scr.cov[x] = cv; if (cv <= 0) coverage_flag = 0; }
        unsigned char c = 4;
        if (((mi != -1) || (!check)) && coverage_flag) c = (mi >= 0 && mi <= 3) ? (unsigned char)mi : 4;
        E.scr.cons[x] = c;
    }
    if (E.tid == 0) E.S->cons_len = n < 0 ? 0 : n;
    FIG_SYNC();
}

FIG_D void fig_copy_str(FigEng &E, unsigned char *dst, int *dlen, const unsigned char *src, int slen) {
    for (int x = E.tid; x < slen; x += E.nt) dst[x] = src[x];
    if (E.tid == 0) *dlen = slen;
    FIG_SYNC();
}

FIG_D bool fig_tlt(const FigTrip &a, const FigTrip &b) { return a.v[0] < b.v[0]; }
FIG_D void fig_tswap(FigTrip &a, FigTrip &b) { FigTrip t = a; a = b; b = t; }

FIG_D void fig_adjust_heap(FigTrip *first, int holeIndex, int len, FigTrip value) {
    int topIndex = holeIndex, secondChild = holeIndex;
    while (secondChild < (len - 1) / 2) {
        secondChild = 2 * (secondChild + 1);
        if (fig_tlt(first[secondChild], first[secondChild - 1])) secondChild--;
        first[holeIndex] = first[secondChild];
        holeIndex = secondChild;
    }
    if ((len & 1) == 0 && secondChild == (len - 2) / 2) {
        secondChild = 2 * (secondChild + 1);
        first[holeIndex] = first[secondChild - 1];
        holeIndex = secondChild - 1;
    }
    int parent = (holeIndex - 1) / 2;
    while (holeIndex > topIndex && fig_tlt(first[parent], value)) {
        first[holeIndex] = first[parent];
        holeIndex = parent;
        parent = (holeIndex - 1) / 2;
    }
    first[holeIndex] = value;
}
FIG_D void fig_heapsort(FigTrip *first, int n) {
    if (n < 2) return;
    for (int parent = (n - 2) / 2;; parent--) { FigTrip v = first[parent]; fig_adjust_heap(first, parent, n, v); if (parent == 0) break; }
    for (int last = n; last > 1; last--) { FigTrip v = first[last - 1]; first[last - 1] = first[0]; fig_adjust_heap(first, 0, last - 1, v); }
}
FIG_D void fig_unguarded_linear_insert(FigTrip *a, int last) {
    FigTrip val = a[last];
    int next = last - 1;
    while (fig_tlt(val, a[next])) { a[last] = a[next]; last = next; next--; }
    a[last] = val;
}
FIG_D void fig_insertion_sort(FigTrip *a, int first, int last) {
    if (first == last) return;
    for (int i = first + 1; i != last; ++i) {
        if (fig_tlt(a[i], a[first])) { FigTrip val = a[i]; for (int k = i; k > first; k--) a[k] = a[k - 1]; a[first] = val; }
        else fig_unguarded_linear_insert(a, i);
    }
}
FIG_D void fig_std_sort(FigTrip *a, int n) {
    if (n <= 0) return;
    int lg = 0; { int t = n; while (t > 1) { t >>= 1; lg++; } }
    int stack_f[64], stack_l[64], stack_d[64], sp = 0;
    stack_f[0] = 0; stack_l[0] = n; stack_d[0] = lg * 2; sp = 1;
    while (sp > 0) {
        sp--;
        int first = stack_f[sp], last = stack_l[sp], depth = stack_d[sp];
        while (last - first > 16) {
            if (depth == 0) { fig_heapsort(a + first, last - first); break; }
            --depth;
            int mid = first + (last - first) / 2;
            {
                int A = first + 1, Bm = mid, C = last - 1;
                if (fig_tlt(a[A], a[Bm])) {
                    if (fig_tlt(a[Bm], a[C])) fig_tswap(a[first], a[Bm]);
                    else if (fig_tlt(a[A], a[C])) fig_tswap(a[first], a[C]);
                    else fig_tswap(a[first], a[A]);
                } else if (fig_tlt(a[A], a[C])) fig_tswap(a[first], a[A]);
                else if (fig_tlt(a[Bm], a[C])) fig_tswap(a[first], a[C]);
                else fig_tswap(a[first], a[Bm]);
            }
            int lo = first + 1, hi = last;
            while (true) {
                while (fig_tlt(a[lo], a[first])) ++lo;
                --hi;
                while (fig_tlt(a[first], a[hi])) --hi;
                if (!(lo < hi)) break;
                fig_tswap(a[lo], a[hi]);
                ++lo;
            }
            int cut = lo;
            if (sp < 63) { stack_f[sp] = first; stack_l[sp] = cut; stack_d[sp] = depth; sp++; }
            first = cut;
        }
    }
    if (n > 16) { fig_insertion_sort(a, 0, 16); for (int i = 16; i != n; ++i) fig_unguarded_linear_insert(a, i); }
    else fig_insertion_sort(a, 0, n);
}

#include "fig_engine_core.h"

#endif
```

figbird_amd/csrc/fig_engine_shared.h:

```cpp
#ifndef FIG_ENGINE_SHARED_H
#define FIG_ENGINE_SHARED_H
#ifndef FIG_EMU
#define FIG_FI __device__ static __forceinline__

FIG_D unsigned fig_wave_max_u32(unsigned v) {
#define FIG_DPP_UMAX(ctrl, rmask) do { const unsigned y_ = (unsigned)__builtin_amdgcn_update_dpp(0, (int)v, ctrl, rmask, 0xf, false); v = y_ > v ? y_ : v; } while (0)
    FIG_DPP_UMAX(0x111, 0xf); FIG_DPP_UMAX(0x112, 0xf); FIG_DPP_UMAX(0x114, 0xf); FIG_DPP_UMAX(0x118, 0xf);
    FIG_DPP_UMAX(0x142, 0xa); FIG_DPP_UMAX(0x143, 0xc);
#undef FIG_DPP_UMAX
    return (unsigned)__builtin_amdgcn_readlane((int)v, 63);
}


template <int N>
FIG_FI void fig_weights_n(const double (&x)[N], double (&w)[N]) {
    double m[N], a[N], b[N], r[N], s[N], z[N], q[N], s_lo[N], t[N], lm_lo[N], ed[N], p_hi[N], p_lo[N], r_hi[N], sum[N], err[N], tl[N];
    int e[N];
#pragma unroll
    for (int i = 0; i < N; i++) { m[i] = __builtin_amdgcn_frexp_mant(x[i]); e[i] = __builtin_amdgcn_frexp_exp(x[i]); }
#pragma unroll
    for (int i = 0; i < N; i++) { const bool lowhalf = m[i] < 0.70710678118654752440; m[i] = lowhalf ? m[i] + m[i] : m[i]; e[i] = lowhalf ? e[i] - 1 : e[i]; }
#pragma unroll
    for (int i = 0; i < N; i++) { a[i] = m[i] - 1.0; b[i] = m[i] + 1.0; }
#pragma unroll
    for (int i = 0; i < N; i++) r[i] = __builtin_amdgcn_rcp(b[i]);
#pragma unroll
    for (int i = 0; i < N; i++) { const double e0 = __builtin_fma(-b[i], r[i], 1.0); r[i] = __builtin_fma(r[i], e0, r[i]); }
#pragma unroll
    for (int i = 0; i < N; i++) { s[i] = a[i] * r[i]; z[i] = s[i] * s[i]; q[i] = 2.0 / 23.0; }
#define FIG_W_H(c) _Pragma("unroll") for (int i = 0; i < N; i++) q[i] = __builtin_fma(q[i], z[i], c);
    FIG_W_H(2.0 / 21.0) FIG_W_H(2.0 / 19.0) FIG_W_H(2.0 / 17.0) FIG_W_H(2.0 / 15.0) FIG_W_H(2.0 / 13.0)
    FIG_W_H(2.0 / 11.0) FIG_W_H(2.0 / 9.0) FIG_W_H(2.0 / 7.0) FIG_W_H(2.0 / 5.0) FIG_W_H(2.0 / 3.0)
#undef FIG_W_H
    const double L2hi = 0x1.34413509f78p-2, L2lo = 0x1.fef311f12b358p-46;
    const double IE_hi = 0x1.bcb7b1526e50ep-2, IE_lo = 0x1.95355baaafad3p-57;
#pragma unroll
    for (int i = 0; i < N; i++) { s_lo[i] = __builtin_fma(-s[i], b[i], a[i]) * r[i]; t[i] = s[i] * z[i] * q[i]; }
#pragma unroll
    for (int i = 0; i < N; i++) { const double lm_hi = 2.0 * s[i]; lm_lo[i] = __builtin_fma(2.0, s_lo[i], t[i]); ed[i] = (double)e[i]; p_hi[i] = lm_hi * IE_hi;
                                  p_lo[i] = __builtin_fma(lm_hi, IE_hi, -p_hi[i]) + __builtin_fma(lm_hi, IE_lo, lm_lo[i] * IE_hi); r_hi[i] = ed[i] * L2hi; }
#pragma unroll
    for (int i = 0; i < N; i++) { sum[i] = r_hi[i] + p_hi[i]; err[i] = (r_hi[i] - sum[i]) + p_hi[i]; if (e[i] == 0) { sum[i] = p_hi[i]; err[i] = 0.0; } }
#pragma unroll
    for (int i = 0; i < N; i++) { const double res = sum[i] + (err[i] + __builtin_fma(ed[i], L2lo, p_lo[i])); tl[i] = x[i] == 0.0 ? -__builtin_inf() : res; }
    const double L2E = 0x1.71547652b82fep+0, LN2_HI = 0x1.62e42fee00000p-1, LN2_LO = 0x1.a39ef35793c76p-33;
    double y[N], kd[N], rh[N], rl[N], rr[N], g[N];
#pragma unroll
    for (int i = 0; i < N; i++) { y[i] = 0.5 * tl[i]; kd[i] = __builtin_rint(y[i] * L2E); }
#pragma unroll
    for (int i = 0; i < N; i++) { rh[i] = __builtin_fma(-kd[i], LN2_HI, y[i]); rl[i] = -kd[i] * LN2_LO; rr[i] = rh[i] + rl[i]; g[i] = 1.0 / 6227020800.0; }
#define FIG_W_H(c) _Pragma("unroll") for (int i = 0; i < N; i++) g[i] = __builtin_fma(g[i], rr[i], c);
    FIG_W_H(1.0 / 479001600.0) FIG_W_H(1.0 / 39916800.0) FIG_W_H(1.0 / 3628800.0) FIG_W_H(1.0 / 362880.0) FIG_W_H(1.0 / 40320.0) FIG_W_H(1.0 / 5040.0)
    FIG_W_H(1.0 / 720.0) FIG_W_H(1.0 / 120.0) FIG_W_H(1.0 / 24.0) FIG_W_H(1.0 / 6.0) FIG_W_H(0.5)
#undef FIG_W_H
#pragma unroll
    for (int i = 0; i < N; i++) {
        const double tt = rr[i] * rr[i] * g[i];
        const double ss = 1.0 + rh[i], ee = (1.0 - ss) + rh[i];
        const double res = __builtin_ldexp(ss + ((ee + rl[i]) + tt), (int)kd[i]);
        w[i] = y[i] < -745.0 ? 0.0 : res;
    }
}

typedef FigState __attribute__((address_space(3))) *fig_lsp;

#define FIG_SH_M2(pa, pb, w) \
    "s_and_b32 m0, " w ", 0xffff\n v_mul_f64 " pa ", v[232:233], " pa "\n" \
    "s_lshr_b32 m0, " w ", 16\n v_mul_f64 " pb ", v[232:233], " pb "\n"
#define FIG_SH_FIN "{v[232:233]}"(f[0]), "{v[234:235]}"(f[1]), "{v[236:237]}"(f[2]), "{v[238:239]}"(f[3]), "{v[240:241]}"(f[4]), \
                   "{v[242:243]}"(f[5]), "{v[244:245]}"(f[6]), "{v[246:247]}"(f[7]), "{v[248:249]}"(one)
FIG_FI void fig_sh_mul4(double *p, const double *f, double one, const uint32_t *w) {
    asm volatile("s_set_gpr_idx_on %[w0], 1\n" FIG_SH_M2("%[p0]", "%[p1]", "%[w0]") FIG_SH_M2("%[p2]", "%[p3]", "%[w1]") "s_set_gpr_idx_off\n"
                 : [p0] "+v"(p[0]), [p1] "+v"(p[1]), [p2] "+v"(p[2]), [p3] "+v"(p[3])
                 : FIG_SH_FIN, [w0] "s"(w[0]), [w1] "s"(w[1]) : "scc");
}
FIG_FI void fig_sh_mul8(double *p, const double *f, double one, const uint32_t *w) {
    asm volatile("s_set_gpr_idx_on %[w0], 1\n" FIG_SH_M2("%[p0]", "%[p1]", "%[w0]") FIG_SH_M2("%[p2]", "%[p3]", "%[w1]")
                 FIG_SH_M2("%[p4]", "%[p5]", "%[w2]") FIG_SH_M2("%[p6]", "%[p7]", "%[w3]") "s_set_gpr_idx_off\n"
                 : [p0] "+v"(p[0]), [p1] "+v"(p[1]), [p2] "+v"(p[2]), [p3] "+v"(p[3]), [p4] "+v"(p[4]), [p5] "+v"(p[5]), [p6] "+v"(p[6]), [p7] "+v"(p[7])
                 : FIG_SH_FIN, [w0] "s"(w[0]), [w1] "s"(w[1]), [w2] "s"(w[2]), [w3] "s"(w[3]) : "scc");
}
FIG_FI void fig_sh_mul16(double *p, const double *f, double one, const uint32_t *w) {
    asm volatile("s_set_gpr_idx_on %[w0], 1\n" FIG_SH_M2("%[p0]", "%[p1]", "%[w0]") FIG_SH_M2("%[p2]", "%[p3]", "%[w1]")
                 FIG_SH_M2("%[p4]", "%[p5]", "%[w2]") FIG_SH_M2("%[p6]", "%[p7]", "%[w3]") FIG_SH_M2("%[p8]", "%[p9]", "%[w4]")
                 FIG_SH_M2("%[p10]", "%[p11]", "%[w5]") FIG_SH_M2("%[p12]", "%[p13]", "%[w6]") FIG_SH_M2("%[p14]", "%[p15]", "%[w7]") "s_set_gpr_idx_off\n"
                 : [p0] "+v"(p[0]), [p1] "+v"(p[1]), [p2] "+v"(p[2]), [p3] "+v"(p[3]), [p4] "+v"(p[4]), [p5] "+v"(p[5]), [p6] "+v"(p[6]), [p7] "+v"(p[7]),
                   [p8] "+v"(p[8]), [p9] "+v"(p[9]), [p10] "+v"(p[10]), [p11] "+v"(p[11]), [p12] "+v"(p[12]), [p13] "+v"(p[13]), [p14] "+v"(p[14]), [p15] "+v"(p[15])
                 : FIG_SH_FIN, [w0] "s"(w[0]), [w1] "s"(w[1]), [w2] "s"(w[2]), [w3] "s"(w[3]), [w4] "s"(w[4]), [w5] "s"(w[5]), [w6] "s"(w[6]), [w7] "s"(w[7])
                 : "scc");
}

template <int NS>
FIG_FI void fig_sh_step(double (&p)[FIG_SH_C], const uint32_t (&wc)[NS / 2], const double (&kc)[4], const FigPQ (&ac)[4],
                        uint32_t (&wn)[NS / 2], double (&kn)[4], FigPQ (&an)[4], const FigPQ *colp, int ncolE, fig_cu32p st, fig_cdp ktf, fig_cdp ktr, int jn) {
    {
        __builtin_amdgcn_s_waitcnt(0xc07f);
        fig_cu32p sn = st + jn * (FIG_SH_C / 2);
#pragma unroll
        for (int k = 0; k < NS / 2; k++) wn[k] = sn[k];
        kn[0] = ktf[2 * jn]; kn[1] = ktf[2 * jn + 1]; kn[2] = ktr[2 * jn]; kn[3] = ktr[2 * jn + 1];
        const FigPQ *cn = colp + jn;
#pragma unroll
        for (int b = 0; b < 4; b++) an[b] = cn[b * ncolE];
    }
    double f[8], m1[8], m2[8];
#pragma unroll
    for (int b = 0; b < 4; b++) { m1[b] = ac[b].p * kc[0]; m1[4 + b] = ac[b].p * kc[2]; }
#pragma unroll
    for (int b = 0; b < 4; b++) { m2[b] = kc[1] * ac[b].q; m2[4 + b] = kc[3] * ac[b].q; }
#pragma unroll
    for (int i = 0; i < 8; i++) f[i] = m1[i] + m2[i];
    const double one = 1.0;
    if (NS == 32) { fig_sh_mul16(&p[0], f, one, &wc[0]); fig_sh_mul16(&p[16], f, one, &wc[8]); }
    else if (NS == 16) fig_sh_mul16(&p[0], f, one, &wc[0]);
    else if (NS == 8) fig_sh_mul8(&p[0], f, one, &wc[0]);
    else fig_sh_mul4(&p[0], f, one, &wc[0]);
}

template <int NS>
FIG_FI void fig_sh_chain(double (&p)[FIG_SH_C], const FigPQ *colp, int ncolE, fig_cu32p st, fig_cdp ktf, fig_cdp ktr, int L) {
    uint32_t w0[NS / 2], w1[NS / 2];
    double k0[4], k1[4];
    FigPQ a0[4], a1[4];
#pragma unroll
    for (int k = 0; k < NS / 2; k++) w0[k] = st[k];
    k0[0] = ktf[0]; k0[1] = ktf[1]; k0[2] = ktr[0]; k0[3] = ktr[1];
#pragma unroll
    for (int b = 0; b < 4; b++) a0[b] = colp[b * ncolE];
    int j = 0;
#ifndef FIG_SH_UNROLL
#define FIG_SH_UNROLL 2
#endif
    for (; j + 2 * FIG_SH_UNROLL <= L; j += 2 * FIG_SH_UNROLL) {
#pragma unroll
        for (int u = 0; u < FIG_SH_UNROLL; u++) {
            fig_sh_step<NS>(p, w0, k0, a0, w1, k1, a1, colp, ncolE, st, ktf, ktr, j + 2 * u + 1);
            fig_sh_step<NS>(p, w1, k1, a1, w0, k0, a0, colp, ncolE, st, ktf, ktr, j + 2 * u + 2);
        }
    }
    for (; j + 2 <= L; j += 2) {
        fig_sh_step<NS>(p, w0, k0, a0, w1, k1, a1, colp, ncolE, st, ktf, ktr, j + 1);
        fig_sh_step<NS>(p, w1, k1, a1, w0, k0, a0, colp, ncolE, st, ktf, ktr, j + 2);
    }
    if (j < L) fig_sh_step<NS>(p, w0, k0, a0, w1, k1, a1, colp, ncolE, st, ktf, ktr, j + 1);
}

template <int NS>
FIG_FI void fig_sh_unit(const int s0, FigState &S, const FigHotU &U, const FigPQ *PQ, fig_cu32p stream, fig_gdp prow, const int pst, const int o, const bool vo, const int ocalc) {
    const fig_lsp SL = (fig_lsp)&S;
    double p[FIG_SH_C];
#pragma unroll
    for (int i = 0; i < NS; i++) {
        const int s = s0 + i;
        const int lo = fig_u(SL->sh_lo[s]), hi = fig_u(SL->sh_hi[s]), tis0 = fig_u(SL->sh_tis0[s]), dir = (fig_u(SL->sh_aux[s]) & 4) ? 1 : -1;
        p[i] = 1.0;
        if (ocalc >= lo && ocalc <= hi) p[i] = ((fig_gcdp)U.insd)[tis0 + dir * ocalc];
    }
    fig_sh_chain<NS>(p, PQ + (ocalc + U.xoff), U.ncolE, stream + ((s0 & (FIG_SH_C - 1)) >> 1), (fig_cdp)U.kt_fwd, (fig_cdp)U.kt_rev, U.L);
    if (vo) {
        fig_gdp dst = prow + (long long)s0 * pst + (o + U.L - 1);
#pragma unroll
        for (int i = 0; i < NS; i++) dst[(long long)i * pst] = p[i];
    }
}

template <int CPL>
FIG_NOINLINE FIG_D void fig_hot_estep_sh(FigEng &E, int gapoffset) {
    constexpr bool LDS = true;
    constexpr int NR = 4;
    constexpr int KP = 2;
    FigState &S = *E.S;
    const fig_lsp SL = (fig_lsp)E.S;
    const FigHotU U = fig_hot_uniforms(E);
    const int G = U.G, nU = U.nU, cg = U.cg;
    const long long ub = U.ub;
    const FigPQ *PQ = fig_pq_ptr<LDS>(E);
    double *W = fig_w_ptr<LDS>(E);
    const int Wcap = U.Wcap;
    const int wave = fig_u(E.wave), lane = E.lane, tid = E.tid, nw = U.nw;
    const fig_cu32p stream0 = (fig_cu32p)(fig_uptr(fig_uptr(E.B)->ustream) + fig_u64(fig_uptr(E.g)->streamOff));
    const long long wbase = nU > 0 ? fig_u64(U.u_woff[ub]) : 0;
    const fig_gdp prow = (fig_gdp)fig_uptr(E.scr.wg);
    const int pst = Wcap;
    double acc[CPL];
#pragma unroll
    for (int m = 0; m < CPL; m++) acc[m] = 0;
    const int pb_c = wave & 3, pb_x0 = (wave >> 2) * CPL * U.wsz + lane;
    unsigned long long fl_acc = 0;
    uint32_t *plb = (uint32_t *)(fig_lds + fig_u(E.off_plb));
    const int Wn = G + U.L - 1;
    const int nT = (Wn + 63) >> 6;
    int scn = fig_u(E.sh_on);
    scn = scn < 1 ? 1 : (scn > FIG_SH_SC ? FIG_SH_SC : scn);
    FIG_SYNC();
    FIG_T0(E);
    for (int c0 = 0; c0 < nU; c0 += scn * FIG_SH_C) {
        const int nrd = nU - c0 < scn * FIG_SH_C ? nU - c0 : scn * FIG_SH_C;
        const int nc = (nrd + FIG_SH_C - 1) / FIG_SH_C;
        if (tid < FIG_SH_SC * FIG_SH_C) {
            const int r = c0 + tid;
            int lo = 0, hi = -1, tis0 = 0, dir = 1; bool irr = false;
            int len = 0, aux = 0; long long woff = 0;
            if (tid < nrd) {
                len = U.u_len[ub + r]; aux = U.u_aux[ub + r]; woff = U.u_woff[ub + r];
                const FigWin w = fig_window_u(U, U.u_pos[ub + r], len, gapoffset);
                lo = w.lo; hi = w.hi; tis0 = w.tis0; dir = w.dir;
                irr = ((aux >> 1) & 1) != 0 || len != U.L;
            }
            SL->sh_lo[tid] = (short)lo; SL->sh_hi[tid] = (short)hi; SL->sh_tis0[tid] = tis0; SL->sh_len[tid] = (unsigned char)len;
            SL->sh_aux[tid] = (unsigned char)((aux & 3) | (dir > 0 ? 4 : 0)); SL->sh_woff[tid] = (unsigned)(woff - wbase);
            const unsigned long long im = fig_ballot(irr);
            if (lane == 0) { SL->sh_irr[2 * wave] = (unsigned)(im & 0xffffffffULL); SL->sh_irr[2 * wave + 1] = (unsigned)(im >> 32); }
        }
        FIG_SYNC();
        uint32_t plv_next = 0;
        if (wave < NR && c0 + wave < nU) {
            const int len = fig_u(SL->sh_len[wave]);
            const int ndw = 2 + ((len + 3) >> 2) + 4;
            if (lane < ndw) plv_next = ((fig_gcu32p)U.packed)[wbase + fig_u((int)SL->sh_woff[wave]) + ((len + 15) >> 4) + ((len + 31) >> 5) + lane];
        }
        FIG_TICK(E, 34);
        {
            const int nit = nT * nc;
            const int nfull = nit / nw, mleft = nit - nfull * nw;
            const fig_cu32p stc = stream0 + (long long)(c0 / FIG_SH_C) * U.L * (FIG_SH_C / 2);
            for (int k = 0; k < nfull; k++) {
                const int it = k * nw + wave, ci = it / nT, tl = it - ci * nT;
                const int ob = -(U.L - 1) + 64 * tl, o = ob + lane;
                const bool vo = o <= G - 1;
                fig_sh_unit<32>(ci * FIG_SH_C, S, U, PQ, stc + (long long)ci * U.L * (FIG_SH_C / 2), prow, pst, o, vo, vo ? o : ob);
            }
            if (mleft > 0) {
                int fsplit = 1;
                while (fsplit * 2 * mleft <= nw && fsplit < 8) fsplit *= 2;
                if (wave < mleft * fsplit) {
                    const int nsl = FIG_SH_C / fsplit;
                    const int it = nfull * nw + wave / fsplit, ci = it / nT, tl = it - ci * nT;
                    const int s0 = ci * FIG_SH_C + (wave % fsplit) * nsl;
                    const int ob = -(U.L - 1) + 64 * tl, o = ob + lane;
                    const bool vo = o <= G - 1;
                    const fig_cu32p stp = stc + (long long)ci * U.L * (FIG_SH_C / 2);
                    if (fsplit == 1) fig_sh_unit<32>(s0, S, U, PQ, stp, prow, pst, o, vo, vo ? o : ob);
                    else if (fsplit == 2) fig_sh_unit<16>(s0, S, U, PQ, stp, prow, pst, o, vo, vo ? o : ob);
                    else if (fsplit == 4) fig_sh_unit<8>(s0, S, U, PQ, stp, prow, pst, o, vo, vo ? o : ob);
                    else fig_sh_unit<4>(s0, S, U, PQ, stp, prow, pst, o, vo, vo ? o : ob);
                }
            }
        }
        FIG_TICK(E, 35);
        FIG_SYNC();
        double pn[NR][KP];
#pragma unroll
        for (int t = 0; t < NR; t++)
#pragma unroll
            for (int k = 0; k < KP; k++) { const int i = tid + k * U.nt; pn[t][k] = (i < Wn && c0 + t < nU) ? prow[(long long)t * pst + i] : 0.0; }
        for (int q0 = 0; q0 < nrd; q0 += NR) {
            const unsigned irr = (unsigned)fig_u((int)SL->sh_irr[q0 >> 5]) >> (q0 & 31);
            int g_lo = 0, g_hi = -1;
            if (lane < NR && c0 + q0 + lane < nU) { g_lo = SL->sh_lo[q0 + lane]; g_hi = SL->sh_hi[q0 + lane]; }
            if (wave < NR) {
                plb[wave * 64 + lane] = plv_next;
                plv_next = 0;
                const int sn = q0 + NR + wave;
                if (sn < nrd) {
                    const int len = fig_u(SL->sh_len[sn]);
                    const int ndw = 2 + ((len + 3) >> 2) + 4;
                    if (lane < ndw) plv_next = ((fig_gcu32p)U.packed)[wbase + fig_u((int)SL->sh_woff[sn]) + ((len + 15) >> 4) + ((len + 31) >> 5) + lane];
                }
            }
            double pc[NR][KP];
#pragma unroll
            for (int t = 0; t < NR; t++)
#pragma unroll
                for (int k = 0; k < KP; k++) pc[t][k] = pn[t][k];
            FIG_TICK(E, 19);
            double wq[NR][KP];
#pragma unroll
            for (int k = 0; k < KP; k++) {
                if (k * U.nt + wave * 64 < Wn) {
                    double px[NR], wx[NR];
#pragma unroll
                    for (int t = 0; t < NR; t++) px[t] = pc[t][k];
                    fig_weights_n<NR>(px, wx);
#pragma unroll
                    for (int t = 0; t < NR; t++) wq[t][k] = wx[t];
                } else {
#pragma unroll
                    for (int t = 0; t < NR; t++) wq[t][k] = 0.0;
                }
            }
#pragma unroll
            for (int t = 0; t < NR; t++) {
                const int s = q0 + t, r = c0 + s;
                if (r >= nU) continue;
                const int lo = __builtin_amdgcn_readlane(g_lo, t), hi = __builtin_amdgcn_readlane(g_hi, t);
                double *wrow = W + (long long)t * Wcap + (U.L - 1);
                const bool isirr = (irr >> t) & 1u;
                if (hi < lo) continue;
                if (!isirr) {
                    double pr = 0.0; int po = FIG_NOPOS;
#pragma unroll
                    for (int k = 0; k < KP; k++) {
                        const int i = tid + k * U.nt, o = i - (U.L - 1);
                        if (k * U.nt + wave * 64 < Wn) {
                            const bool in = i < Wn && o >= lo && o <= hi;
                            if (i < Wn) wrow[o] = in ? wq[t][k] : 0.0;
                            if (in) {
                                fl_acc += 4ULL * (unsigned long long)U.L + (unsigned long long)fig_ovl(o, U.L, G);
                                if (pc[t][k] > pr) { pr = pc[t][k]; po = o; }
                            }
                        }
                    }
                    FIG_TICK(E, 20);
                    long long bits; memcpy(&bits, &pr, 8);
                    const unsigned hi32 = (unsigned)((unsigned long long)bits >> 32), lo32 = (unsigned)((unsigned long long)bits & 0xffffffffULL);
                    const unsigned mh = fig_wave_max_u32(hi32);
                    const unsigned long long ah = fig_ballot(hi32 == mh);
                    const unsigned ml = (ah & (ah - 1)) == 0ULL ? (unsigned)fig_lane_read_i32((int)lo32, fig_ctz64(ah)) : fig_wave_max_u32(hi32 == mh ? lo32 : 0u);
                    const unsigned long long am = fig_ballot(po != FIG_NOPOS && hi32 == mh && lo32 == ml);
                    const bool any = (mh | ml) != 0u && am != 0ULL;
                    const int ao = any ? fig_lane_read_i32(po, fig_ctz64(am)) : FIG_NOPOS;
                    if (lane == 0) {
                        const unsigned long long mb = ((unsigned long long)mh << 32) | ml;
                        double mv; memcpy(&mv, &mb, 8);
                        SL->wv_v[t * 8 + wave] = any ? mv : 0.0; SL->wv_o[t * 8 + wave] = ao;
                    }
                    FIG_TICK(E, 21);
                } else {
                    FigReadS rs; rs.len = fig_u(SL->sh_len[s]); rs.rev = fig_u(SL->sh_aux[s]) & 1; rs.hasN = 1; rs.pos = 0; rs.woff = wbase + fig_u((int)SL->sh_woff[s]);
                    fig_cu32p pk = (fig_cu32p)(U.packed + rs.woff);
                    const int nw2 = (rs.len + 15) >> 4;
                    fig_cdp kt = (fig_cdp)(rs.rev ? U.kt_rev + 2 * (U.L - rs.len) : U.kt_fwd);
                    const double *Q4 = fig_q4_ptr<LDS>(E);
                    const int tis0 = fig_u(SL->sh_tis0[s]), dir = (fig_u(SL->sh_aux[s]) & 4) ? 1 : -1;
                    for (int i = -(U.L - 1) + tid; i < G; i += U.nt) if (i < lo || i > hi) wrow[i] = 0.0;
                    FigBest best; best.v = -FIG_DBL_MAX; best.o = FIG_NOPOS;
                    unsigned long long nplace = 0, nadd = 0;
                    for (int o = lo + tid; o <= hi; o += U.nt) {
                        const double pr = fig_hot_chain_e<LDS>(PQ, Q4, U.ncolE, pk, nw2, kt, rs.len, 0, false, o + U.xoff, U.insd[tis0 + dir * o]);
                        const double tl = fig_log10(pr);
                        if (tl > best.v) { best.v = tl; best.o = o; }
                        wrow[o] = fig_exp(0.5 * tl);
                        nplace++; nadd += fig_ovl(o, rs.len, G);
                    }
                    fl_acc += 4ULL * nplace * (unsigned long long)rs.len + nadd;
                    const double bv = fig_wave_max_dpp(best.o == FIG_NOPOS ? -FIG_DBL_MAX : best.v);
                    const unsigned long long am = fig_ballot(best.o != FIG_NOPOS && best.v == bv);
                    const int ao = am ? fig_lane_read_i32(best.o, fig_ctz64(am)) : FIG_NOPOS;
                    if (lane == 0) { SL->wv_v[t * 8 + wave] = bv; SL->wv_o[t * 8 + wave] = bv > -FIG_DBL_MAX ? ao : FIG_NOPOS; }
                }
            }
            FIG_TICK(E, 36);
            FIG_SYNC();
            FIG_TICK(E, 37);
            if (q0 + NR < nrd) {
#pragma unroll
                for (int t = 0; t < NR; t++)
#pragma unroll
                    for (int k = 0; k < KP; k++) { const int i = tid + k * U.nt; pn[t][k] = (i < Wn && c0 + q0 + NR + t < nU) ? prow[(long long)(q0 + NR + t) * pst + i] : 0.0; }
            }
            if (tid >= 64 && tid < 64 + NR) {
                const int t = tid - 64, s = q0 + t;
                if (c0 + s < nU) {
                    FigBest b; b.v = -FIG_DBL_MAX; b.o = FIG_NOPOS;
                    if (SL->sh_hi[s] >= SL->sh_lo[s]) for (int k = 0; k < nw; k++) { FigBest y; y.v = SL->wv_v[t * 8 + k]; y.o = SL->wv_o[t * 8 + k]; b = fig_best_merge(b, y); }
                    if (b.o != FIG_NOPOS) E.scr.maxlv[c0 + s] = b.v;
                    else { E.scr.maxlv[c0 + s] = 0; fig_atomic_add_i32(&S.invalid_count, 1); }
                    E.scr.hint_e[c0 + s] = b.o;
                }
            }
            FIG_TICK(E, 27);
            uint32_t plv_nx = plb[lane];
            for (int t = 0; t < NR && c0 + q0 + t < nU; t++) {
                if (U.nw == 8) { if ((t + (wave >> 2)) & 1) __builtin_amdgcn_s_setprio(1); else __builtin_amdgcn_s_setprio(0); }
                const uint32_t plv = plv_nx;
                if (t + 1 < NR) plv_nx = plb[(t + 1) * 64 + lane];
                const int lo = __builtin_amdgcn_readlane(g_lo, t), hi = __builtin_amdgcn_readlane(g_hi, t);
                if (hi < lo) continue;
                const double *wrow = W + (long long)t * Wcap + (U.L - 1);
                const uint32_t cw0 = (uint32_t)__builtin_amdgcn_readlane((int)plv, 0), cw1 = (uint32_t)__builtin_amdgcn_readlane((int)plv, 1);
                const int nA = (int)(cw0 & 255), nC = (int)((cw0 >> 8) & 255), nG = (int)((cw0 >> 16) & 255), nT_ = (int)(cw0 >> 24);
                const int n4 = (int)(cw1 & 255);
                const int dC = 2 + ((nA + 3) >> 2), dG = dC + ((nC + 3) >> 2), dT = dG + ((nG + 3) >> 2), d4 = dT + ((nT_ + 3) >> 2);
                const int n = pb_c == 0 ? nA : pb_c == 1 ? nC : pb_c == 2 ? nG : nT_;
                const int d0 = pb_c == 0 ? 2 : pb_c == 1 ? dC : pb_c == 2 ? dG : dT;
                const double *wl = wrow + pb_x0;
                int k4 = 0;
                FIG_TICK(E, 28); FIG_COUNT(E, 31, 1); FIG_COUNT(E, 32, n * CPL);
                for (; k4 + 1 <= (n >> 2); k4++) {
                    const uint32_t s4 = (uint32_t)__builtin_amdgcn_readlane((int)plv, d0 + k4);
                    const double *p0 = wl - (int)(s4 & 255), *p1 = wl - (int)((s4 >> 8) & 255), *p2 = wl - (int)((s4 >> 16) & 255), *p3 = wl - (int)(s4 >> 24);
                    if (CPL <= 4) {
                        double w0[CPL], w1[CPL], w2[CPL], w3[CPL];
#pragma unroll
                        for (int i = 0; i < CPL; i++) { w0[i] = FIG_LDV(p0 + i * 64); w1[i] = FIG_LDV(p1 + i * 64); w2[i] = FIG_LDV(p2 + i * 64); w3[i] = FIG_LDV(p3 + i * 64); }
#pragma unroll
                        for (int i = 0; i < CPL; i++) acc[i] += w0[i];
#pragma unroll
                        for (int i = 0; i < CPL; i++) acc[i] += w1[i];
#pragma unroll
                        for (int i = 0; i < CPL; i++) acc[i] += w2[i];
#pragma unroll
                        for (int i = 0; i < CPL; i++) acc[i] += w3[i];
                    } else {
                        double w0[CPL], w1[CPL];
#pragma unroll
                        for (int i = 0; i < CPL; i++) { w0[i] = FIG_LDV(p0 + i * 64); w1[i] = FIG_LDV(p1 + i * 64); }
#pragma unroll
                        for (int i = 0; i < CPL; i++) acc[i] += w0[i];
#pragma unroll
                        for (int i = 0; i < CPL; i++) { w0[i] = FIG_LDV(p2 + i * 64); acc[i] += w1[i]; }
#pragma unroll
                        for (int i = 0; i < CPL; i++) { w1[i] = FIG_LDV(p3 + i * 64); acc[i] += w0[i]; }
#pragma unroll
                        for (int i = 0; i < CPL; i++) acc[i] += w1[i];
                    }
                }
                FIG_TICK(E, 29);
                if (n & 3) {
                    const uint32_t s4 = (uint32_t)__builtin_amdgcn_readlane((int)plv, d0 + k4);
                    const int rem = n & 3;
                    const double *p0 = wl - (int)(s4 & 255), *p1 = wl - (int)((s4 >> 8) & 255), *p2 = wl - (int)((s4 >> 16) & 255);
                    double w0[CPL], w1[CPL], w2[CPL];
#pragma unroll
                    for (int i = 0; i < CPL; i++) { w0[i] = FIG_LDV(p0 + i * 64); w1[i] = FIG_LDV(p1 + i * 64); w2[i] = FIG_LDV(p2 + i * 64); }
#pragma unroll
                    for (int i = 0; i < CPL; i++) acc[i] += w0[i];
                    if (rem > 1) {
#pragma unroll
                        for (int i = 0; i < CPL; i++) acc[i] += w1[i];
                    }
                    if (rem > 2) {
#pragma unroll
                        for (int i = 0; i < CPL; i++) acc[i] += w2[i];
                    }
                }
                if (n4 > 0) {
                    for (int x = tid; x < G; x += U.nt) {
                        double a = E.scr.cnt[4 * cg + x];
                        for (int k = 0; k < n4; k++) {
                            const uint32_t s4 = (uint32_t)__builtin_amdgcn_readlane((int)plv, d4 + (k >> 2));
                            a += wrow[x - (int)((s4 >> ((k & 3) * 8)) & 255)];
                        }
                        E.scr.cnt[4 * cg + x] = a;
                    }
                }
                FIG_TICK(E, 30);
            }
            if (U.nw == 8) __builtin_amdgcn_s_setprio(0);
            FIG_TICK(E, 38);
            FIG_SYNC();
            FIG_TICK(E, 39);
        }
        if (tid < nrd) {
            const bool isirr = (SL->sh_irr[tid >> 5] >> (tid & 31)) & 1u;
            if (!isirr && E.scr.hint_e[c0 + tid] != FIG_NOPOS) E.scr.maxlv[c0 + tid] = fig_log10(E.scr.maxlv[c0 + tid]);
        }
    }
#pragma unroll
    for (int i = 0; i < CPL; i++) {
        const int x = pb_x0 + i * U.wsz;
        if (x < G) E.scr.cnt[pb_c * cg + x] = acc[i];
    }
    E.flops += fl_acc;
    FIG_SYNC();
}

FIG_D bool fig_sh_applies(const FigEng &E, int cpl) {
    if (!E.sh_on || E.tiles > 0 || !E.pq_lds || E.nteams < 4 || cpl > 8 || cpl < 1) return false;
    if (!E.B->ustream || E.M->L < 32) return false;
    const FigState &S = *E.S;
    if (S.left < E.xoff) return false;
    const int Wn = S.G + E.M->L - 1;
    return Wn <= 2 * E.nt && (E.nw == 4 || E.nw == 8) && (long long)FIG_SH_SC * FIG_SH_C * E.Wcap <= (long long)E.B->capW;
}

#endif
#endif
```

figbird_amd/csrc/fig_types.h:

```cpp
#ifndef FIG_TYPES_H
#define FIG_TYPES_H
#include <stdint.h>

#define FIG_MAX_READLEN 200
#define FIG_READ_CAP 3000
#define FIG_MAX_GAP 100000
#define FIG_FLANK 208
#define FIG_DBL_MAX 1.7976931348623157e308
#define FIG_SH_C 32
#define FIG_SH_SC 4
#define FIG_SH_ONE 16
#define FIG_MLE_FB 208
#define FIG_TILED_MLE_DOUBLES(ncolE, nw) (7LL * (ncolE) + (long long)(nw) * FIG_MLE_FB + ((ncolE) + 15) / 16 + 16 + 8)

enum { FIG_ORG_NONE = 0, FIG_ORG_FINAL = 1, FIG_ORG_ORIGINAL = 2, FIG_ORG_TIEBREAK = 4 };

enum { FIG_GAP_FINISHED = 0, FIG_GAP_MORE = 1, FIG_GAP_LOOP_DONE = 2 };
struct FigGapCtl { int32_t status, j, range, reach; };

struct alignas(16) FigItem { int32_t gap, j, slot, pad; };
struct alignas(16) FigEntry { int32_t gap, n, pad0, pad1; };
static_assert(sizeof(FigGapCtl) == 16 && sizeof(FigItem) == 16 && sizeof(FigEntry) == 16, "control words are four int32: buffers and copies are sized by sizeof");

enum FigCounter {
    FIG_CNT_PLACE = 0,
    FIG_CNT_FLOPS = 1, FIG_CNT_SPEC = 2,
    FIG_CNT_MLE_ALG = 3, FIG_CNT_MLE_EXEC = 4,
    FIG_CNT_PROF_LO = 8, FIG_CNT_WAIT = 30, FIG_CNT_WAVE = 31, FIG_CNT_PROF_HI = 32,
    FIG_CNT_N = 64
};
#define FIG_PROF_SLOTS 40
#define FIG_PROF_SPLIT 22

struct FigDevModel {
    int32_t L;
    int32_t Tmin, Tmax, cutoff;
    int32_t partial_flag, unmapped, script_itr, D, read_length, neg_overlap, partial_len, unm_limit;
    int32_t max_insert;
    double T[25];
    const double *e;
    const double *ome;
    const double *ome1;
    const double *m3;
    const double *insd;
    const double *qtab;
    double fmm_up;
};

struct FigDevGap {
    int64_t gapStart, contigLen;
    int32_t G0, stat2, stat3, fillflag;
    int32_t nU; int32_t nP;
    int64_t uBase, pBase;
    int32_t alloc_arg; float gpf1, gpf2; int32_t lgf;
    int64_t flankOff;
    int64_t strOff;
    int32_t gapNo; int32_t cls;
    int64_t persistOff;
    int32_t capGg, rangeCap, nslots, pad;
    int64_t streamOff;
};

struct FigDevReads {
    const int32_t *pos;
    const int32_t *aux;
    const int32_t *clip;
    const int32_t *refpos;
    const int32_t *len;
    const int64_t *woff;
    const int64_t *qoff;
};

struct FigDevBatch {
    int64_t n_gaps;
    const FigDevGap *gaps;
    const int32_t *order;
    FigDevReads u, p;
    const uint32_t *packed;
    const uint32_t *ustream;
    const uint8_t *qual;
    const uint8_t *flank;
    int32_t *filled_len, *gaptofill; char *str;
    int32_t dbg_max_cand; int32_t *dbg_n_cand; int32_t *dbg_cand_i; double *dbg_cand_lik; int32_t *dbg_n_place;
    int32_t *draw_pos, *draw_isz, *draw_len; int64_t n_ureads;
    int32_t dbg_plane_cols, dbg_plane_reads; double *dbg_counts, *dbg_read_maxlv;
    int32_t *queue_head;
    unsigned long long *counters;
    uint8_t *scratch; int64_t scratch_stride;
    int32_t capG, capR, capP, capC;
    int32_t capW, capE;
    uint8_t *persist;
    FigGapCtl *gapctl;
    const uint8_t *ot_preset;
    int32_t *sup_counts, *sup_origin;
};

#endif
```

Baseline: 23.97.

## Sort reads by orientation so shared-factor units can skip the unused strand

Reads within each shared-factor chunk are reordered so forward-strand reads come first and reverse-strand reads follow. The mapping is built on device in both the stream-packing kernel and the fill kernel. Each 32-slot unit then runs a forward-only, reverse-only or mixed variant, so pure units skip half of the factor multiplies and k-table loads. In exchange it adds a slot-mapping pass with extra syncs in the stream kernel, an indirection through the row map, and per-mode template instantiations that raise code size and register pressure. New counters record how many units ran in each mode.

```diff
diff --git a/figbird_amd/csrc/fig_abi.hip b/figbird_amd/csrc/fig_abi.hip
--- a/figbird_amd/csrc/fig_abi.hip
+++ b/figbird_amd/csrc/fig_abi.hip
@@ -30,6 +30,7 @@
     fig_eng_ident(E, threadIdx.x, blockDim.x, 64);
     E.M = &M; E.B = &B;
     E.flops = 0; E.mle_alg = 0; E.mle_exec = 0; E.wait_cycles = 0;
+    E.sh_units[0] = E.sh_units[1] = E.sh_units[2] = 0;
     for (int i = 0; i < FIG_PROF_SLOTS; i++) E.prof[i] = 0;
     unsigned char *slab = B.scratch + (long long)blockIdx.x * B.scratch_stride;
     fig_scratch_layout(slab, B.capG, B.capR, B.capP, B.capC, B.capW, B.capE, &work);
@@ -67,6 +68,7 @@
     if (E.flops) atomicAdd(&B.counters[FIG_CNT_FLOPS], E.flops);
     if (E.mle_alg) atomicAdd(&B.counters[FIG_CNT_MLE_ALG], E.mle_alg);
     if (E.lane == 0 && E.mle_exec) atomicAdd(&B.counters[FIG_CNT_MLE_EXEC], E.mle_exec);
+    if (E.lane == 0) for (int k = 0; k < 3; k++) if (E.sh_units[k]) atomicAdd(&B.counters[FIG_CNT_SH_FWD + k], (unsigned long long)E.sh_units[k]);
 }
 
 template <bool LDS_TAB, int NT>
@@ -122,30 +124,47 @@
     fig_kernel_flush(E, B);
 }
 
-__global__ void __launch_bounds__(256) fig_stream_kernel(FigDevModel M, FigDevBatch B, uint32_t *out) {
+__global__ void __launch_bounds__(256) fig_stream_kernel(FigDevModel M, FigDevBatch B, uint32_t *out, int sh_on, int orient) {
+    __shared__ unsigned char rev_of[FIG_SH_SC * FIG_SH_C], row_of[FIG_SH_SC * FIG_SH_C];
+    const int scn = sh_on < 1 ? 1 : (sh_on > FIG_SH_SC ? FIG_SH_SC : sh_on);
+    const int L = M.L;
     for (long long gi = blockIdx.x; gi < B.n_gaps; gi += gridDim.x) {
         const FigDevGap &g = B.gaps[gi];
-        const int L = M.L;
-        const long long n = (long long)((g.nU + FIG_SH_C - 1) / FIG_SH_C) * L * (FIG_SH_C / 2);
-        for (long long i = threadIdx.x; i < n; i += blockDim.x) {
-            const int sp = (int)(i % (FIG_SH_C / 2));
-            const long long cj = i / (FIG_SH_C / 2);
-            const int j = (int)(cj % L);
-            uint32_t v = 0;
-            for (int h = 0; h < 2; h++) {
-                const long long r = (cj / L) * FIG_SH_C + 2 * sp + h;
-                unsigned e = 0x1000u | FIG_SH_ONE;
-                if (r < g.nU) {
-                    const long long idx = g.uBase + r;
-                    const int len = B.u.len[idx], aux = B.u.aux[idx];
-                    if (len == L && !(aux & 2)) {
-                        const uint32_t w = B.packed[B.u.woff[idx] + (j >> 4)];
-                        e = 0x1000u | (2u * (4u * (unsigned)(aux & 1) + ((w >> ((j & 15) * 2)) & 3u)));
+        for (int c0 = 0; c0 < g.nU; c0 += scn * FIG_SH_C) {
+            const int nrd = g.nU - c0 < scn * FIG_SH_C ? g.nU - c0 : scn * FIG_SH_C;
+            const int t = (int)threadIdx.x;
+            __syncthreads();
+            if (t < nrd) rev_of[t] = (unsigned char)(B.u.aux[g.uBase + c0 + t] & 1);
+            __syncthreads();
+            if (t < nrd) {
+                int fb = 0, nfwd = 0;
+                for (int r = 0; r < nrd; r++) { const int f = !rev_of[r]; nfwd += f; if (r < t) fb += f; }
+                row_of[orient ? fig_sh_slot_of(t, fb, nfwd, rev_of[t]) : t] = (unsigned char)t;
+            }
+            __syncthreads();
+            const int nc = (nrd + FIG_SH_C - 1) / FIG_SH_C;
+            const long long base = g.streamOff + (long long)(c0 / FIG_SH_C) * L * (FIG_SH_C / 2);
+            const int n = nc * L * (FIG_SH_C / 2);
+            for (int i = t; i < n; i += (int)blockDim.x) {
+                const int sp = i % (FIG_SH_C / 2);
+                const int cj = i / (FIG_SH_C / 2);
+                const int j = cj % L;
+                uint32_t v = 0;
+                for (int h = 0; h < 2; h++) {
+                    const int slot = (cj / L) * FIG_SH_C + 2 * sp + h;
+                    unsigned e = 0x1000u | FIG_SH_ONE;
+                    if (slot < nrd) {
+                        const long long idx = g.uBase + c0 + row_of[slot];
+                        const int len = B.u.len[idx], aux = B.u.aux[idx];
+                        if (len == L && !(aux & 2)) {
+                            const uint32_t w = B.packed[B.u.woff[idx] + (j >> 4)];
+                            e = 0x1000u | (2u * (4u * (unsigned)(aux & 1) + ((w >> ((j & 15) * 2)) & 3u)));
+                        }
                     }
+                    v |= e << (16 * h);
                 }
-                v |= e << (16 * h);
+                out[base + i] = v;
             }
-            out[g.streamOff + i] = v;
         }
     }
 }
@@ -185,6 +204,7 @@
     std::vector<FigLane> lanes;
     fig_stats stats;
     int sh_on = FIG_SH_SC;
+    int sh_orient = 1;
     std::vector<uint8_t> h_ot;
     uint8_t *d_ot = nullptr;
 };
@@ -236,7 +256,7 @@
         return FIG_EHIP;
     }
     memset(&ctx->stats, 0, sizeof(ctx->stats));
-    ctx->sh_on = fig_knobs_from_env(0).sh_on;
+    { const FigKnobs k = fig_knobs_from_env(0); ctx->sh_on = k.sh_on; ctx->sh_orient = k.sh_orient; }
     *out = ctx;
     return FIG_OK;
 }
@@ -302,7 +322,7 @@
 
 template <bool LDS_TAB, int NT>
 static hipError_t launch_kind(fig_ctx *ctx, const fig_ctx::Cls &c, const FigDevBatch &db, hipStream_t stream, FigKind kind, int blocks, const void *list, int n, int qsel) {
-    const FigKernArgs A = fig_kargs_of(c.c, qsel, ctx->sh_on);
+    const FigKernArgs A = fig_kargs_of(c.c, qsel, ctx->sh_on, ctx->sh_orient);
     switch (kind) {
         case FIG_K_FILL: return launch_one(fig_fill_kernel<LDS_TAB, NT>, c.c.lds, NT, blocks, stream, ctx->dm, db, A);
         case FIG_K_BEGIN: return launch_one(fig_begin_kernel<LDS_TAB, NT>, c.c.lds, NT, blocks, stream, ctx->dm, db, A);
@@ -365,7 +385,7 @@
         db.ustream = (const uint32_t *)p;
         FIG_HIP(hipMemsetD32Async((hipDeviceptr_t)p, (int)(((0x1000u | FIG_SH_ONE) << 16) | (0x1000u | FIG_SH_ONE)), (size_t)K.stream_total, ctx->stream));
         if (ng > 0) {
-            hipLaunchKernelGGL(fig_stream_kernel, dim3((unsigned)std::min<int64_t>(ng, 4096)), dim3(256), 0, ctx->stream, ctx->dm, db, (uint32_t *)p);
+            hipLaunchKernelGGL(fig_stream_kernel, dim3((unsigned)std::min<int64_t>(ng, 4096)), dim3(256), 0, ctx->stream, ctx->dm, db, (uint32_t *)p, ctx->sh_on, ctx->sh_orient);
             FIG_HIP(hipGetLastError());
         }
     }
@@ -574,6 +594,7 @@
       fprintf(stderr, "[figprof] raw slots:"); for (int i = 0; i < FIG_PROF_SLOTS; i++) fprintf(stderr, " %d:%.1f", i, prof(i) / 1e9); fprintf(stderr, "\n");
       fprintf(stderr, "[figprof] barrier wait %.3f of %.3f wave-Gcycles = %.1f %%\n", cnt[FIG_CNT_WAIT] / 1e9, wave / 1e9, wave ? 100.0 * cnt[FIG_CNT_WAIT] / wave : 0.0); }
 #endif
+    if (knobs.log) fprintf(stderr, "[figsched] shared-factor phase-A units: fwd=%llu rev=%llu both=%llu\n", cnt[FIG_CNT_SH_FWD], cnt[FIG_CNT_SH_REV], cnt[FIG_CNT_SH_BOTH]);
     if (knobs.log) fprintf(stderr, "[figsched] useful flops %.4g, speculative evaluations executed %.4g (%.1f %% discarded)\n", (double)cnt[FIG_CNT_FLOPS], (double)cnt[FIG_CNT_SPEC], cnt[FIG_CNT_SPEC] ? 100.0 * (1.0 - ((double)cnt[FIG_CNT_FLOPS] / (double)cnt[FIG_CNT_SPEC])) : 0.0);
     fig_stats_from_counters(cnt, ctx->stats);
     int rc = fig_compact_results(ng, hstr.data(), ctx->h_str_off.data(), out);
diff --git a/figbird_amd/csrc/fig_abi_host.h b/figbird_amd/csrc/fig_abi_host.h
--- a/figbird_amd/csrc/fig_abi_host.h
+++ b/figbird_amd/csrc/fig_abi_host.h
@@ -118,12 +118,12 @@
     st.mle_alg_flops = (double)cnt[FIG_CNT_MLE_ALG]; st.mle_exec_flops = (double)cnt[FIG_CNT_MLE_EXEC];
 }
 
-static FigKernArgs fig_kargs_of(const FigLaunchClass &c, int qsel, int sh_on) {
+static FigKernArgs fig_kargs_of(const FigLaunchClass &c, int qsel, int sh_on, int sh_orient = 0) {
     FigKernArgs A;
     A.capG = c.capG; A.capGl = c.capGl; A.ncolE = c.ncolE; A.Wcap = c.Wcap; A.nteams = c.nteams;
     A.q_begin = c.q_begin; A.q_end = c.q_end; A.qsel = qsel;
     A.tiles = c.tiles; A.tile_step = c.tile_step; A.tile_cols = c.tile_cols; A.tiled_max = c.tiled_max;
-    A.sh_on = sh_on;
+    A.sh_on = sh_on; A.sh_orient = sh_orient;
     return A;
 }
 
@@ -173,18 +173,20 @@
     int minc;
     double ipw;
     int sh_on;
+    int sh_orient;
 };
 
 static FigKnobs fig_knobs_from_env(int unmapped) {
     FigKnobs k;
     const char *sched = getenv("FIG_SCHED"), *ser = getenv("FIG_LANES"), *mc = getenv("FIG_MIN_CHUNK"), *ipw = getenv("FIG_ITEMS_PER_WG");
-    const char *ev = getenv("FIG_ESTEP"), *sc = getenv("FIG_SH_CHUNKS");
+    const char *ev = getenv("FIG_ESTEP"), *sc = getenv("FIG_SH_CHUNKS"), *so = getenv("FIG_SH_ORIENT");
     k.seq = sched && strcmp(sched, "seq") == 0;
     k.lanes_serial = ser && strcmp(ser, "serial") == 0;
     k.log = getenv("FIG_SCHED_LOG") != nullptr;
     k.minc = mc ? std::max(1, atoi(mc)) : 16;
     k.ipw = ipw ? std::max(1.0, atof(ipw)) : (unmapped ? 12.0 : 6.0);
     k.sh_on = (ev && !strcmp(ev, "pair")) ? 0 : (sc ? std::max(1, std::min(FIG_SH_SC, atoi(sc))) : FIG_SH_SC);
+    k.sh_orient = (so && !strcmp(so, "0")) ? 0 : 1;
     return k;
 }
 
diff --git a/figbird_amd/csrc/fig_engine.h b/figbird_amd/csrc/fig_engine.h
--- a/figbird_amd/csrc/fig_engine.h
+++ b/figbird_amd/csrc/fig_engine.h
@@ -2,6 +2,7 @@
 #define FIG_ENGINE_H
 
 #include "fig_types.h"
+#include "fig_orient.h"
 
 #ifdef FIG_EMU
 #include <cmath>
@@ -119,6 +120,7 @@
     int sh_tis0[FIG_SH_SC * FIG_SH_C];
     unsigned sh_woff[FIG_SH_SC * FIG_SH_C];
     unsigned char sh_len[FIG_SH_SC * FIG_SH_C], sh_aux[FIG_SH_SC * FIG_SH_C];
+    unsigned char sh_row[FIG_SH_SC * FIG_SH_C];
     unsigned sh_irr[16], sh_pad;
     int mle_next, pad_mn;
     int fin_i[8];
@@ -225,6 +227,8 @@
     double *wbuf;
     int Wcap, nteams;
     int sh_on;
+    int sh_orient;
+    unsigned sh_units[3];
     int lane, wave, nw, wsz;
     const double *kt_fwd, *kt_rev;
     const double *mt_fwd, *mt_rev;
@@ -244,11 +248,11 @@
     E.lane = (int)(tid % wsz); E.wave = (int)(tid / wsz); E.nw = (int)((nt + wsz - 1) / wsz); E.wsz = (int)wsz;
 }
 
-struct FigKernArgs { int capG, capGl, ncolE, Wcap, nteams, q_begin, q_end, qsel, tiles, tile_step, tile_cols, tiled_max, sh_on; };
+struct FigKernArgs { int capG, capGl, ncolE, Wcap, nteams, q_begin, q_end, qsel, tiles, tile_step, tile_cols, tiled_max, sh_on, sh_orient; };
 
 FIG_D long long fig_eng_carve(FigEng &E, const FigDevModel &M, const FigKernArgs &A, bool lds_tab) {
     E.capG = A.capG;
-    E.ncolE = A.ncolE; E.xoff = M.L - 1; E.Wcap = A.Wcap; E.nteams = A.nteams; E.sh_on = A.sh_on;
+    E.ncolE = A.ncolE; E.xoff = M.L - 1; E.Wcap = A.Wcap; E.nteams = A.nteams; E.sh_on = A.sh_on; E.sh_orient = A.sh_orient;
     long long off = 0;
     E.pq_lds = lds_tab; E.w_lds = lds_tab;
     E.tiles = A.tiles; E.tile_step = A.tile_step; E.tile_cols = A.tile_cols;
diff --git a/figbird_amd/csrc/fig_engine_shared.h b/figbird_amd/csrc/fig_engine_shared.h
--- a/figbird_amd/csrc/fig_engine_shared.h
+++ b/figbird_amd/csrc/fig_engine_shared.h
@@ -69,6 +69,8 @@
     "s_lshr_b32 m0, " w ", 16\n v_mul_f64 " pb ", v[232:233], " pb "\n"
 #define FIG_SH_FIN "{v[232:233]}"(f[0]), "{v[234:235]}"(f[1]), "{v[236:237]}"(f[2]), "{v[238:239]}"(f[3]), "{v[240:241]}"(f[4]), \
                    "{v[242:243]}"(f[5]), "{v[244:245]}"(f[6]), "{v[246:247]}"(f[7]), "{v[248:249]}"(one)
+#define FIG_SH_FIN_F "{v[232:233]}"(f[0]), "{v[234:235]}"(f[1]), "{v[236:237]}"(f[2]), "{v[238:239]}"(f[3]), "{v[248:249]}"(one)
+#define FIG_SH_FIN_R "{v[240:241]}"(f[4]), "{v[242:243]}"(f[5]), "{v[244:245]}"(f[6]), "{v[246:247]}"(f[7]), "{v[248:249]}"(one)
 FIG_FI void fig_sh_mul4(double *p, const double *f, double one, const uint32_t *w) {
     asm volatile("s_set_gpr_idx_on %[w0], 1\n" FIG_SH_M2("%[p0]", "%[p1]", "%[w0]") FIG_SH_M2("%[p2]", "%[p3]", "%[w1]") "s_set_gpr_idx_off\n"
                  : [p0] "+v"(p[0]), [p1] "+v"(p[1]), [p2] "+v"(p[2]), [p3] "+v"(p[3])
@@ -80,17 +82,22 @@
                  : [p0] "+v"(p[0]), [p1] "+v"(p[1]), [p2] "+v"(p[2]), [p3] "+v"(p[3]), [p4] "+v"(p[4]), [p5] "+v"(p[5]), [p6] "+v"(p[6]), [p7] "+v"(p[7])
                  : FIG_SH_FIN, [w0] "s"(w[0]), [w1] "s"(w[1]), [w2] "s"(w[2]), [w3] "s"(w[3]) : "scc");
 }
+#define FIG_SH_MUL16(FIN) \
+    asm volatile("s_set_gpr_idx_on %[w0], 1\n" FIG_SH_M2("%[p0]", "%[p1]", "%[w0]") FIG_SH_M2("%[p2]", "%[p3]", "%[w1]") \
+                 FIG_SH_M2("%[p4]", "%[p5]", "%[w2]") FIG_SH_M2("%[p6]", "%[p7]", "%[w3]") FIG_SH_M2("%[p8]", "%[p9]", "%[w4]") \
+                 FIG_SH_M2("%[p10]", "%[p11]", "%[w5]") FIG_SH_M2("%[p12]", "%[p13]", "%[w6]") FIG_SH_M2("%[p14]", "%[p15]", "%[w7]") "s_set_gpr_idx_off\n" \
+                 : [p0] "+v"(p[0]), [p1] "+v"(p[1]), [p2] "+v"(p[2]), [p3] "+v"(p[3]), [p4] "+v"(p[4]), [p5] "+v"(p[5]), [p6] "+v"(p[6]), [p7] "+v"(p[7]), \
+                   [p8] "+v"(p[8]), [p9] "+v"(p[9]), [p10] "+v"(p[10]), [p11] "+v"(p[11]), [p12] "+v"(p[12]), [p13] "+v"(p[13]), [p14] "+v"(p[14]), [p15] "+v"(p[15]) \
+                 : FIN, [w0] "s"(w[0]), [w1] "s"(w[1]), [w2] "s"(w[2]), [w3] "s"(w[3]), [w4] "s"(w[4]), [w5] "s"(w[5]), [w6] "s"(w[6]), [w7] "s"(w[7]) \
+                 : "scc")
+template <int MODE>
 FIG_FI void fig_sh_mul16(double *p, const double *f, double one, const uint32_t *w) {
-    asm volatile("s_set_gpr_idx_on %[w0], 1\n" FIG_SH_M2("%[p0]", "%[p1]", "%[w0]") FIG_SH_M2("%[p2]", "%[p3]", "%[w1]")
-                 FIG_SH_M2("%[p4]", "%[p5]", "%[w2]") FIG_SH_M2("%[p6]", "%[p7]", "%[w3]") FIG_SH_M2("%[p8]", "%[p9]", "%[w4]")
-                 FIG_SH_M2("%[p10]", "%[p11]", "%[w5]") FIG_SH_M2("%[p12]", "%[p13]", "%[w6]") FIG_SH_M2("%[p14]", "%[p15]", "%[w7]") "s_set_gpr_idx_off\n"
-                 : [p0] "+v"(p[0]), [p1] "+v"(p[1]), [p2] "+v"(p[2]), [p3] "+v"(p[3]), [p4] "+v"(p[4]), [p5] "+v"(p[5]), [p6] "+v"(p[6]), [p7] "+v"(p[7]),
-                   [p8] "+v"(p[8]), [p9] "+v"(p[9]), [p10] "+v"(p[10]), [p11] "+v"(p[11]), [p12] "+v"(p[12]), [p13] "+v"(p[13]), [p14] "+v"(p[14]), [p15] "+v"(p[15])
-                 : FIG_SH_FIN, [w0] "s"(w[0]), [w1] "s"(w[1]), [w2] "s"(w[2]), [w3] "s"(w[3]), [w4] "s"(w[4]), [w5] "s"(w[5]), [w6] "s"(w[6]), [w7] "s"(w[7])
-                 : "scc");
-}
-
-template <int NS>
+    if constexpr (MODE == FIG_SH_FWD) FIG_SH_MUL16(FIG_SH_FIN_F);
+    else if constexpr (MODE == FIG_SH_REV) FIG_SH_MUL16(FIG_SH_FIN_R);
+    else FIG_SH_MUL16(FIG_SH_FIN);
+}
+
+template <int NS, int MODE>
 FIG_FI void fig_sh_step(double (&p)[FIG_SH_C], const uint32_t (&wc)[NS / 2], const double (&kc)[4], const FigPQ (&ac)[4],
                         uint32_t (&wn)[NS / 2], double (&kn)[4], FigPQ (&an)[4], const FigPQ *colp, int ncolE, fig_cu32p st, fig_cdp ktf, fig_cdp ktr, int jn) {
     {
@@ -98,33 +105,45 @@
         fig_cu32p sn = st + jn * (FIG_SH_C / 2);
 #pragma unroll
         for (int k = 0; k < NS / 2; k++) wn[k] = sn[k];
-        kn[0] = ktf[2 * jn]; kn[1] = ktf[2 * jn + 1]; kn[2] = ktr[2 * jn]; kn[3] = ktr[2 * jn + 1];
+        if (MODE & FIG_SH_FWD) { kn[0] = ktf[2 * jn]; kn[1] = ktf[2 * jn + 1]; }
+        if (MODE & FIG_SH_REV) { kn[2] = ktr[2 * jn]; kn[3] = ktr[2 * jn + 1]; }
         const FigPQ *cn = colp + jn;
 #pragma unroll
         for (int b = 0; b < 4; b++) an[b] = cn[b * ncolE];
     }
     double f[8], m1[8], m2[8];
-#pragma unroll
-    for (int b = 0; b < 4; b++) { m1[b] = ac[b].p * kc[0]; m1[4 + b] = ac[b].p * kc[2]; }
-#pragma unroll
-    for (int b = 0; b < 4; b++) { m2[b] = kc[1] * ac[b].q; m2[4 + b] = kc[3] * ac[b].q; }
-#pragma unroll
-    for (int i = 0; i < 8; i++) f[i] = m1[i] + m2[i];
+    if constexpr (MODE == FIG_SH_BOTH) {
+#pragma unroll
+        for (int b = 0; b < 4; b++) { m1[b] = ac[b].p * kc[0]; m1[4 + b] = ac[b].p * kc[2]; }
+#pragma unroll
+        for (int b = 0; b < 4; b++) { m2[b] = kc[1] * ac[b].q; m2[4 + b] = kc[3] * ac[b].q; }
+#pragma unroll
+        for (int i = 0; i < 8; i++) f[i] = m1[i] + m2[i];
+    } else {
+        constexpr int fo = MODE == FIG_SH_REV ? 4 : 0, ko = MODE == FIG_SH_REV ? 2 : 0;
+#pragma unroll
+        for (int b = 0; b < 4; b++) m1[fo + b] = ac[b].p * kc[ko];
+#pragma unroll
+        for (int b = 0; b < 4; b++) m2[fo + b] = kc[ko + 1] * ac[b].q;
+#pragma unroll
+        for (int b = 0; b < 4; b++) f[fo + b] = m1[fo + b] + m2[fo + b];
+    }
     const double one = 1.0;
-    if (NS == 32) { fig_sh_mul16(&p[0], f, one, &wc[0]); fig_sh_mul16(&p[16], f, one, &wc[8]); }
-    else if (NS == 16) fig_sh_mul16(&p[0], f, one, &wc[0]);
+    if (NS == 32) { fig_sh_mul16<MODE>(&p[0], f, one, &wc[0]); fig_sh_mul16<MODE>(&p[16], f, one, &wc[8]); }
+    else if (NS == 16) fig_sh_mul16<MODE>(&p[0], f, one, &wc[0]);
     else if (NS == 8) fig_sh_mul8(&p[0], f, one, &wc[0]);
     else fig_sh_mul4(&p[0], f, one, &wc[0]);
 }
 
-template <int NS>
+template <int NS, int MODE>
 FIG_FI void fig_sh_chain(double (&p)[FIG_SH_C], const FigPQ *colp, int ncolE, fig_cu32p st, fig_cdp ktf, fig_cdp ktr, int L) {
     uint32_t w0[NS / 2], w1[NS / 2];
     double k0[4], k1[4];
     FigPQ a0[4], a1[4];
 #pragma unroll
     for (int k = 0; k < NS / 2; k++) w0[k] = st[k];
-    k0[0] = ktf[0]; k0[1] = ktf[1]; k0[2] = ktr[0]; k0[3] = ktr[1];
+    if (MODE & FIG_SH_FWD) { k0[0] = ktf[0]; k0[1] = ktf[1]; }
+    if (MODE & FIG_SH_REV) { k0[2] = ktr[0]; k0[3] = ktr[1]; }
 #pragma unroll
     for (int b = 0; b < 4; b++) a0[b] = colp[b * ncolE];
     int j = 0;
@@ -134,34 +153,93 @@
     for (; j + 2 * FIG_SH_UNROLL <= L; j += 2 * FIG_SH_UNROLL) {
 #pragma unroll
         for (int u = 0; u < FIG_SH_UNROLL; u++) {
-            fig_sh_step<NS>(p, w0, k0, a0, w1, k1, a1, colp, ncolE, st, ktf, ktr, j + 2 * u + 1);
-            fig_sh_step<NS>(p, w1, k1, a1, w0, k0, a0, colp, ncolE, st, ktf, ktr, j + 2 * u + 2);
+            fig_sh_step<NS, MODE>(p, w0, k0, a0, w1, k1, a1, colp, ncolE, st, ktf, ktr, j + 2 * u + 1);
+            fig_sh_step<NS, MODE>(p, w1, k1, a1, w0, k0, a0, colp, ncolE, st, ktf, ktr, j + 2 * u + 2);
         }
     }
     for (; j + 2 <= L; j += 2) {
-        fig_sh_step<NS>(p, w0, k0, a0, w1, k1, a1, colp, ncolE, st, ktf, ktr, j + 1);
-        fig_sh_step<NS>(p, w1, k1, a1, w0, k0, a0, colp, ncolE, st, ktf, ktr, j + 2);
-    }
-    if (j < L) fig_sh_step<NS>(p, w0, k0, a0, w1, k1, a1, colp, ncolE, st, ktf, ktr, j + 1);
+        fig_sh_step<NS, MODE>(p, w0, k0, a0, w1, k1, a1, colp, ncolE, st, ktf, ktr, j + 1);
+        fig_sh_step<NS, MODE>(p, w1, k1, a1, w0, k0, a0, colp, ncolE, st, ktf, ktr, j + 2);
+    }
+    if (j < L) fig_sh_step<NS, MODE>(p, w0, k0, a0, w1, k1, a1, colp, ncolE, st, ktf, ktr, j + 1);
 }
 
 template <int NS>
-FIG_FI void fig_sh_unit(const int s0, FigState &S, const FigHotU &U, const FigPQ *PQ, fig_cu32p stream, fig_gdp prow, const int pst, const int o, const bool vo, const int ocalc) {
+FIG_FI void fig_sh_unit(const int s0, FigState &S, const FigHotU &U, const FigPQ *PQ, fig_cu32p stream, fig_gdp prow, const int pst, const int o, const bool vo, const int ocalc,
+                        const int lane, const bool orient, unsigned (&nu)[3]) {
     const fig_lsp SL = (fig_lsp)&S;
+    const int li = lane & (NS - 1);
+    const int rowv = SL->sh_row[s0 + li];
+    const int lov = SL->sh_lo[rowv], hiv = SL->sh_hi[rowv], tisv = SL->sh_tis0[rowv], auxv = SL->sh_aux[rowv];
+    int mode = FIG_SH_BOTH;
+    if (NS == FIG_SH_C && orient) mode = fig_sh_mode(fig_ballot((auxv & 1) != 0), fig_ballot((auxv & 8) != 0));
+    nu[0] += mode == FIG_SH_FWD; nu[1] += mode == FIG_SH_REV; nu[2] += mode == FIG_SH_BOTH;
     double p[FIG_SH_C];
 #pragma unroll
     for (int i = 0; i < NS; i++) {
-        const int s = s0 + i;
-        const int lo = fig_u(SL->sh_lo[s]), hi = fig_u(SL->sh_hi[s]), tis0 = fig_u(SL->sh_tis0[s]), dir = (fig_u(SL->sh_aux[s]) & 4) ? 1 : -1;
+        const int lo = __builtin_amdgcn_readlane(lov, i), hi = __builtin_amdgcn_readlane(hiv, i), tis0 = __builtin_amdgcn_readlane(tisv, i);
+        const int dir = (__builtin_amdgcn_readlane(auxv, i) & 4) ? 1 : -1;
         p[i] = 1.0;
         if (ocalc >= lo && ocalc <= hi) p[i] = ((fig_gcdp)U.insd)[tis0 + dir * ocalc];
     }
-    fig_sh_chain<NS>(p, PQ + (ocalc + U.xoff), U.ncolE, stream + ((s0 & (FIG_SH_C - 1)) >> 1), (fig_cdp)U.kt_fwd, (fig_cdp)U.kt_rev, U.L);
+    const FigPQ *colp = PQ + (ocalc + U.xoff);
+    const fig_cu32p st = stream + ((s0 & (FIG_SH_C - 1)) >> 1);
+    if constexpr (NS == FIG_SH_C) {
+        if (mode == FIG_SH_FWD) fig_sh_chain<NS, FIG_SH_FWD>(p, colp, U.ncolE, st, (fig_cdp)U.kt_fwd, (fig_cdp)U.kt_rev, U.L);
+        else if (mode == FIG_SH_REV) fig_sh_chain<NS, FIG_SH_REV>(p, colp, U.ncolE, st, (fig_cdp)U.kt_fwd, (fig_cdp)U.kt_rev, U.L);
+        else fig_sh_chain<NS, FIG_SH_BOTH>(p, colp, U.ncolE, st, (fig_cdp)U.kt_fwd, (fig_cdp)U.kt_rev, U.L);
+    } else {
+        fig_sh_chain<NS, FIG_SH_BOTH>(p, colp, U.ncolE, st, (fig_cdp)U.kt_fwd, (fig_cdp)U.kt_rev, U.L);
+    }
+    int rows = SL->sh_row[s0 + li];
+    asm volatile("" : "+v"(rows));
     if (vo) {
-        fig_gdp dst = prow + (long long)s0 * pst + (o + U.L - 1);
-#pragma unroll
-        for (int i = 0; i < NS; i++) dst[(long long)i * pst] = p[i];
-    }
+        const fig_gdp dst = prow + (o + U.L - 1);
+#pragma unroll
+        for (int i = 0; i < NS; i++) dst[(long long)(__builtin_amdgcn_readlane(rows, i) & (FIG_SH_SC * FIG_SH_C - 1)) * pst] = p[i];
+    }
+}
+
+FIG_NOINLINE FIG_D void fig_sh_phase_a(FigEng &E, const int c0_, const int nrd_) {
+    FigState &S = *E.S;
+    const FigHotU U = fig_hot_uniforms(E);
+    const int c0 = fig_u(c0_), nrd = fig_u(nrd_);
+    const int G = U.G, nw = U.nw, wave = fig_u(E.wave), lane = E.lane;
+    const FigPQ *PQ = fig_pq_ptr<true>(E);
+    const fig_cu32p stream0 = (fig_cu32p)(fig_uptr(fig_uptr(E.B)->ustream) + fig_u64(fig_uptr(E.g)->streamOff));
+    const fig_gdp prow = (fig_gdp)fig_uptr(E.scr.wg);
+    const int pst = U.Wcap;
+    const int nT = (G + U.L - 1 + 63) >> 6, nc = (nrd + FIG_SH_C - 1) / FIG_SH_C;
+    const int nit = nT * nc;
+    const bool orient = fig_u(E.sh_orient) != 0;
+    unsigned nu[3] = {0, 0, 0};
+    const int nfull = nit / nw, mleft = nit - nfull * nw;
+    const fig_cu32p stc = stream0 + (long long)(c0 / FIG_SH_C) * U.L * (FIG_SH_C / 2);
+    int fsplit = 1;
+    while (mleft > 0 && fsplit * 2 * mleft <= nw && fsplit < 8) fsplit *= 2;
+    const int nwhole = nfull + ((mleft > 0 && fsplit == 1) ? 1 : 0);
+    for (int k = 0; k < nwhole; k++) {
+        const int it = k * nw + wave, ci = it / nT, tl = it - ci * nT;
+        if (it >= nit) break;
+        const int ob = -(U.L - 1) + 64 * tl, o = ob + lane;
+        const bool vo = o <= G - 1;
+        fig_sh_unit<32>(ci * FIG_SH_C, S, U, PQ, stc + (long long)ci * U.L * (FIG_SH_C / 2), prow, pst, o, vo, vo ? o : ob, lane, orient, nu);
+    }
+    if (mleft > 0 && fsplit > 1) {
+        if (wave < mleft * fsplit) {
+            const int nsl = FIG_SH_C / fsplit;
+            const int it = nfull * nw + wave / fsplit, ci = it / nT, tl = it - ci * nT;
+            const int s0 = ci * FIG_SH_C + (wave % fsplit) * nsl;
+            const int ob = -(U.L - 1) + 64 * tl, o = ob + lane;
+            const bool vo = o <= G - 1;
+            const fig_cu32p stp = stc + (long long)ci * U.L * (FIG_SH_C / 2);
+            if (fsplit == 2) fig_sh_unit<16>(s0, S, U, PQ, stp, prow, pst, o, vo, vo ? o : ob, lane, orient, nu);
+            else if (fsplit == 4) fig_sh_unit<8>(s0, S, U, PQ, stp, prow, pst, o, vo, vo ? o : ob, lane, orient, nu);
+            else fig_sh_unit<4>(s0, S, U, PQ, stp, prow, pst, o, vo, vo ? o : ob, lane, orient, nu);
+        }
+    }
+#pragma unroll
+    for (int k = 0; k < 3; k++) E.sh_units[k] += nu[k];
 }
 
 template <int CPL>
@@ -178,7 +256,6 @@
     double *W = fig_w_ptr<LDS>(E);
     const int Wcap = U.Wcap;
     const int wave = fig_u(E.wave), lane = E.lane, tid = E.tid, nw = U.nw;
-    const fig_cu32p stream0 = (fig_cu32p)(fig_uptr(fig_uptr(E.B)->ustream) + fig_u64(fig_uptr(E.g)->streamOff));
     const long long wbase = nU > 0 ? fig_u64(U.u_woff[ub]) : 0;
     const fig_gdp prow = (fig_gdp)fig_uptr(E.scr.wg);
     const int pst = Wcap;
@@ -196,11 +273,13 @@
     FIG_T0(E);
     for (int c0 = 0; c0 < nU; c0 += scn * FIG_SH_C) {
         const int nrd = nU - c0 < scn * FIG_SH_C ? nU - c0 : scn * FIG_SH_C;
-        const int nc = (nrd + FIG_SH_C - 1) / FIG_SH_C;
         if (tid < FIG_SH_SC * FIG_SH_C) {
             const int r = c0 + tid;
             int lo = 0, hi = -1, tis0 = 0, dir = 1; bool irr = false;
-            int len = 0, aux = 0; long long woff = 0;
+            const bool orient = fig_u(E.sh_orient) != 0;
+            int len = 0, aux = 0, aux2 = 1; long long woff = 0;
+            const int tid2 = tid ^ 64;
+            if (orient && tid2 < nrd) aux2 = U.u_aux[ub + c0 + tid2];
             if (tid < nrd) {
                 len = U.u_len[ub + r]; aux = U.u_aux[ub + r]; woff = U.u_woff[ub + r];
                 const FigWin w = fig_window_u(U, U.u_pos[ub + r], len, gapoffset);
@@ -208,7 +287,15 @@
                 irr = ((aux >> 1) & 1) != 0 || len != U.L;
             }
             SL->sh_lo[tid] = (short)lo; SL->sh_hi[tid] = (short)hi; SL->sh_tis0[tid] = tis0; SL->sh_len[tid] = (unsigned char)len;
-            SL->sh_aux[tid] = (unsigned char)((aux & 3) | (dir > 0 ? 4 : 0)); SL->sh_woff[tid] = (unsigned)(woff - wbase);
+            SL->sh_aux[tid] = (unsigned char)((aux & 3) | (dir > 0 ? 4 : 0) | ((tid < nrd && !irr) ? 8 : 0)); SL->sh_woff[tid] = (unsigned)(woff - wbase);
+            int slot = tid;
+            if (orient) {
+                const unsigned long long fme = fig_ballot(tid < nrd && !(aux & 1)), fmo = fig_ballot(tid2 < nrd && !(aux2 & 1));
+                const int nme = __builtin_popcountll(fme), nmo = __builtin_popcountll(fmo);
+                const int before = __builtin_popcountll(fme & ((1ULL << lane) - 1ULL)) + (wave ? nmo : 0);
+                if (tid < nrd) slot = fig_sh_slot_of(tid, before, nme + nmo, aux & 1);
+            }
+            SL->sh_row[slot] = (unsigned char)tid;
             const unsigned long long im = fig_ballot(irr);
             if (lane == 0) { SL->sh_irr[2 * wave] = (unsigned)(im & 0xffffffffULL); SL->sh_irr[2 * wave + 1] = (unsigned)(im >> 32); }
         }
@@ -220,33 +307,7 @@
             if (lane < ndw) plv_next = ((fig_gcu32p)U.packed)[wbase + fig_u((int)SL->sh_woff[wave]) + ((len + 15) >> 4) + ((len + 31) >> 5) + lane];
         }
         FIG_TICK(E, 34);
-        {
-            const int nit = nT * nc;
-            const int nfull = nit / nw, mleft = nit - nfull * nw;
-            const fig_cu32p stc = stream0 + (long long)(c0 / FIG_SH_C) * U.L * (FIG_SH_C / 2);
-            for (int k = 0; k < nfull; k++) {
-                const int it = k * nw + wave, ci = it / nT, tl = it - ci * nT;
-                const int ob = -(U.L - 1) + 64 * tl, o = ob + lane;
-                const bool vo = o <= G - 1;
-                fig_sh_unit<32>(ci * FIG_SH_C, S, U, PQ, stc + (long long)ci * U.L * (FIG_SH_C / 2), prow, pst, o, vo, vo ? o : ob);
-            }
-            if (mleft > 0) {
-                int fsplit = 1;
-                while (fsplit * 2 * mleft <= nw && fsplit < 8) fsplit *= 2;
-                if (wave < mleft * fsplit) {
-                    const int nsl = FIG_SH_C / fsplit;
-                    const int it = nfull * nw + wave / fsplit, ci = it / nT, tl = it - ci * nT;
-                    const int s0 = ci * FIG_SH_C + (wave % fsplit) * nsl;
-                    const int ob = -(U.L - 1) + 64 * tl, o = ob + lane;
-                    const bool vo = o <= G - 1;
-                    const fig_cu32p stp = stc + (long long)ci * U.L * (FIG_SH_C / 2);
-                    if (fsplit == 1) fig_sh_unit<32>(s0, S, U, PQ, stp, prow, pst, o, vo, vo ? o : ob);
-                    else if (fsplit == 2) fig_sh_unit<16>(s0, S, U, PQ, stp, prow, pst, o, vo, vo ? o : ob);
-                    else if (fsplit == 4) fig_sh_unit<8>(s0, S, U, PQ, stp, prow, pst, o, vo, vo ? o : ob);
-                    else fig_sh_unit<4>(s0, S, U, PQ, stp, prow, pst, o, vo, vo ? o : ob);
-                }
-            }
-        }
+        fig_sh_phase_a(E, c0, nrd);
         FIG_TICK(E, 35);
         FIG_SYNC();
         double pn[NR][KP];
diff --git a/figbird_amd/csrc/fig_orient.h b/figbird_amd/csrc/fig_orient.h
--- /dev/null
+++ b/figbird_amd/csrc/fig_orient.h
@@ -0,0 +1,40 @@
+#ifndef FIG_ORIENT_H
+#define FIG_ORIENT_H
+
+#if defined(__HIPCC__) || defined(__CUDACC__)
+#define FIG_ORIENT_FN __host__ __device__ static inline
+#else
+#define FIG_ORIENT_FN static inline
+#endif
+
+enum { FIG_SH_FWD = 1, FIG_SH_REV = 2, FIG_SH_BOTH = 3 };
+
+FIG_ORIENT_FN int fig_sh_slot_of(int r, int fwd_before, int nfwd, int reverse) {
+    return reverse ? nfwd + (r - fwd_before) : fwd_before;
+}
+
+FIG_ORIENT_FN void fig_sh_slot_map(const unsigned char *aux, int nrd, int orient, unsigned char *row_of_slot) {
+    int nfwd = 0;
+    for (int r = 0; r < nrd; r++) nfwd += !(aux[r] & 1);
+    for (int r = 0, fb = 0; r < nrd; r++) {
+        row_of_slot[orient ? fig_sh_slot_of(r, fb, nfwd, aux[r] & 1) : r] = (unsigned char)r;
+        fb += !(aux[r] & 1);
+    }
+}
+
+FIG_ORIENT_FN int fig_sh_mode(unsigned long long rev, unsigned long long reg) {
+    const bool f = (reg & ~rev) != 0, r = (reg & rev) != 0;
+    return f && r ? FIG_SH_BOTH : (r ? FIG_SH_REV : FIG_SH_FWD);
+}
+
+FIG_ORIENT_FN int fig_sh_unit_mode(const unsigned char *aux, const unsigned char *row_of_slot, int nrd, int s0, int ns) {
+    unsigned long long rev = 0, reg = 0;
+    for (int i = 0; i < ns && s0 + i < nrd; i++) {
+        const unsigned char a = aux[row_of_slot[s0 + i]];
+        if (a & 1) rev |= 1ULL << i;
+        if (!(a & 2)) reg |= 1ULL << i;
+    }
+    return fig_sh_mode(rev, reg);
+}
+
+#endif
diff --git a/figbird_amd/csrc/fig_types.h b/figbird_amd/csrc/fig_types.h
--- a/figbird_amd/csrc/fig_types.h
+++ b/figbird_amd/csrc/fig_types.h
@@ -26,6 +26,7 @@
     FIG_CNT_PLACE = 0,
     FIG_CNT_FLOPS = 1, FIG_CNT_SPEC = 2,
     FIG_CNT_MLE_ALG = 3, FIG_CNT_MLE_EXEC = 4,
+    FIG_CNT_SH_FWD = 5, FIG_CNT_SH_REV = 6, FIG_CNT_SH_BOTH = 7,
     FIG_CNT_PROF_LO = 8, FIG_CNT_WAIT = 30, FIG_CNT_WAVE = 31, FIG_CNT_PROF_HI = 32,
     FIG_CNT_N = 64
 };
```

Result: no change. 24.13, median of 6 (+0.6%).
